# lucidrains/audiolm-pytorch

Measured on AMD Instinct MI355X. Metric: audio-tokens/sec fwd+bwd, CoarseTransformer d=1024 seq=2048, higher is better.
Workload: dtype bf16; 1 GPU; CoarseTransformer dim=1024 depth=6 heads=8 (MQA) num_coarse_quantizers=3 codebook=1024 semantic=500 residual_streams=4 flash_attn=True; per-GPU B=8, N=2048 (509 semantic + 512x3 coarse ids + eos/start); mask_prob=0.15; global_batch=8, seq_len=2048, parallelism=dp1

## Files before the change

audiolm-pytorch_amd/_lib.py:

```python
from __future__ import annotations

import ctypes
import os
from ctypes import c_float, c_int, c_longlong, c_ulonglong, c_void_p

_HERE = os.path.dirname(os.path.abspath(__file__))
LIB_PATH = os.environ.get('ALM_LIB_PATH') or os.path.join(_HERE, 'libaudiolm_hip.so')

_P, _I, _L, _F, _U = c_void_p, c_int, c_longlong, c_float, c_ulonglong

SIGNATURES = {
    'alm_gemm_bf16_nt': [_P, _P, _P, _P, _I, _I, _I, _L, _L, _L, _I, _I, _L, _L, _L, _L, _L, _L, _F, _I, _I, _P],
    'alm_gemm_bf16_nt_ws': [_P, _P, _P, _P, _I, _I, _I, _L, _L, _L, _I, _I, _L, _L, _L, _L, _L, _L, _F, _I, _I, _P, _L, _P],
    'alm_gemm_bf16_nt_inl': [_P, _P, _P, _P, _I, _I, _I, _L, _L, _L, _F, _I, _I, _I, _P, _L, _P],
    'alm_gemm_nt_plan': [_I, _I, _I, _I, _I, _P],
    'alm_gemm_nt_ws_bytes': [],
    'alm_gemm_splitk_slices': [_I, _I, _I, _I],
    'alm_gemm_splitk_ws_floats': [_I, _I, _I, _I],
    'alm_gemm_splitk_tile': [_I, _I, _I, _I],
    'alm_gemm_nt_tile_choice': [_I, _I, _I],
    'alm_gemm_tn_batched_plan': [_I, _I, _I, _I, _P],
    'alm_gemm_bf16_nt_splitk': [_P, _P, _P, _P, _I, _I, _I, _L, _L, _L, _I, _L, _L, _L, _F, _I, _P],
    'alm_gemm_bf16_tn_splitk': [_P, _P, _P, _P, _I, _I, _I, _L, _L, _L, _I, _L, _L, _L, _F, _I, _P],
    'alm_gemm_bf16_tn_batched': [_P, _P, _P, _P, _I, _I, _I, _L, _L, _L, _I, _I, _L, _L, _L, _L, _L, _L, _F, _I, _P],
    'alm_gemm_bf16_nt_group2': [_P, _P, _P, _I, _I, _I, _L, _L, _L, _P, _P, _P, _I, _I, _I, _L, _L, _L, _I, _P],
    'alm_gemm_bf16_nt_tile': [_P, _P, _P, _P, _I, _I, _I, _L, _L, _L, _F, _I, _I, _I, _P],
    'alm_transpose_bf16': [_P, _P, _I, _I, _L, _L, _I, _P],
    'alm_transpose_bf16_batched': [_P, _P, _I, _I, _L, _L, _I, _I, _L, _L, _P],
    'alm_pack_weights_multi': [_P, _I, _P],
    'alm_pack_weight': [_P, _I, _I, _L, _P, _L, _I, _I, _P, _L, _P],
    'alm_ln_partial_blocks': [_I],
    'alm_layernorm_fwd': [_P, _I, _L, _P, _P, _I, _L, _P, _L, _P, _P, _I, _I, _P],
    'alm_layernorm_bwd': [_P, _I, _L, _P, _I, _L, _P, _P, _P, _P, _L, _P, _I, _L, _P, _I, _I, _P],
    'alm_colsum': [_P, _I, _L, _I, _I, _P, _F, _I, _P, _P],
    'alm_colsum_chunks': [_I],
    'alm_colsum_partial': [_P, _L, _I, _I, _P, _P],
    'alm_geglu_fwd': [_P, _P, _L, _I, _P],
    'alm_geglu_bwd': [_P, _P, _P, _L, _I, _P],
    'alm_geglu_partial_blocks': [_I],
    'alm_geglu_ln_fwd': [_P, _L, _I, _P, _P, _L, _P, _P, _I, _I, _I, _P],
    'alm_geglu_ln_bwd': [_P, _L, _P, _L, _I, _P, _P, _P, _P, _P, _I, _I, _I, _P],
    'alm_mqa_attn_fwd': [_P, _L, _P, _L, _P, _L, _P, _P, _L, _P, _I, _I, _I, _I, _F, _F, _U, _P, _P],
    'alm_mqa_attn_bwd': [_P, _L, _P, _L, _P, _L, _P, _P, _L, _P, _P, _L, _P, _L, _P, _P, _L, _L, _P, _I, _I, _I, _I, _F, _F, _U, _P, _P],
    'alm_mqa_attn_bias_fwd': [_P, _L, _P, _L, _P, _L, _P, _P, _L, _P, _I, _I, _I, _I, _F, _P, _I, _P, _P, _P, _P, _F, _U, _P, _P],
    'alm_mqa_attn_bias_bwd': [_P, _L, _P, _L, _P, _L, _P, _P, _L, _P, _P, _L, _P, _L, _P, _P, _L, _L, _P, _I, _I, _I, _I, _F,
                              _P, _I, _P, _P, _P, _P, _P, _F, _U, _P, _P],
    'alm_attn_bias_part_rows': [_I, _I, _I],
    'alm_attn_bias_grad_reduce': [_P, _P, _I, _I, _I, _I, _F, _P],
    'alm_posmlp_in_fwd': [_P, _P, _P, _P, _P, _I, _I, _I, _P],
    'alm_posmlp_in_bwd_chunks': [_I],
    'alm_posmlp_in_bwd': [_P, _P, _P, _I, _I, _I, _P],
    'alm_silu_fwd': [_P, _P, _L, _P],
    'alm_silu_bwd': [_P, _P, _P, _L, _P],
    'alm_posmlp_out_fwd': [_P, _P, _P, _P, _P, _I, _I, _I, _F, _P],
    'alm_posmlp_out_bwd': [_P, _P, _P, _P, _P, _P, _I, _I, _I, _I, _F, _P],
    'alm_xattn_softmax_fwd': [_P, _L, _P, _P, _F, _P, _L, _P, _P, _P, _L, _I, _I, _I, _I, _I, _P],
    'alm_xattn_dbias': [_P, _L, _P, _L, _P, _P, _L, _I, _I, _I, _I, _P],
    'alm_xattn_combine': [_P, _L, _P, _P, _P, _L, _L, _I, _I, _P],
    'alm_xattn_softmax_bwd': [_P, _L, _P, _L, _P, _F, _P, _L, _I, _I, _I, _I, _P],
    'alm_xattn_delta': [_P, _L, _P, _L, _P, _I, _I, _I, _I, _P],
    'alm_value_residual_mix': [_P, _L, _P, _L, _P, _L, _L, _I, _P],
    'alm_kv_grad_pack': [_P, _P, _L, _I, _L, _P, _P, _L, _L, _I, _I, _P],
    'alm_forgetful_mask': [_P, _L, _P, _L, _I, _I, _I, _P],
    'alm_coarse_prepare': [_P, _L, _P, _L, _I, _I, _I, _L, _L, _L, _I, _I, _P, _P, _P, _P, _I, _P],
    'alm_semantic_prepare': [_P, _L, _I, _I, _L, _L, _P, _P, _I, _P],
    'alm_unique_consecutive_i64': [_P, _L, _I, _I, _I, _L, _L, _P, _L, _P, _P],
    'alm_fine_prepare': [_P, _L, _P, _L, _I, _I, _I, _L, _L, _I, _I, _I, _P, _P, _P],
    'alm_loss_combine': [_P, _P, _P, _P, _P, _P, _P, _P, _L, _L, _L, _L, _F, _F, _F, _F, _I, _L, _P, _P, _P],
    'alm_mqa_head_groups': [_I],
    'alm_mqa_bwd_parts': [_I, _I, _I],
    'alm_hc_coef_width': [_I],
    'alm_hc_partial_width': [_I, _I],
    'alm_hc_grads_width': [_I, _I],
    'alm_hc_partial_rows': [_I, _I, _I, _I, _L, _I],
    'alm_hc_fwd': [_P, _I, _I, _P, _L, _P, _P, _P, _P, _P, _P, _P, _P, _P, _P, _P, _L, _P, _L, _P, _P, _P, _P, _P, _I, _I, _I, _I, _I, _P],
    'alm_hc_bwd': [_P, _I, _I, _P, _L, _P, _L, _P, _L, _P, _P, _P, _P, _I, _P, _P, _P, _P, _P, _P, _P, _P, _P, _F, _P, _P, _L, _P, _P, _L, _P, _I, _I, _I, _I, _I, _P],
    'alm_hc_param_grads': [_P, _I, _P, _P, _P, _P, _I, _I, _P],
    'alm_hc_param_grads_batched': [_P, _P, _I, _P, _P, _P, _P, _P, _I, _I, _P],
    'alm_streams_expand': [_P, _P, _I, _I, _L, _P],
    'alm_streams_reduce': [_P, _P, _I, _I, _L, _P],
    'alm_residual_add': [_P, _P, _L, _P, _L, _I, _P],
    'alm_f32_to_bf16': [_P, _P, _P, _L, _L, _I, _P],
    'alm_add_f32': [_P, _P, _P, _L, _F, _P],
    'alm_embed_assemble': [_P, _P, _I, _P, _P, _P, _L, _I, _P, _P],
    'alm_embed_scatter_add': [_P, _P, _I, _P, _P, _P, _F, _L, _I, _P],
    'alm_embed_scatter_ws_floats': [_P, _I, _L, _I],
    'alm_embed_scatter_owned': [_P, _P, _I, _P, _P, _P, _F, _L, _I, _P, _P],
    'alm_gather_split_bf16': [_P, _L, _L, _P, _P, _P, _L, _L, _I, _P],
    'alm_gather_rows_bf16': [_P, _L, _P, _P, _L, _L, _I, _P],
    'alm_scatter_rows_bf16': [_P, _L, _P, _P, _L, _L, _I, _P],
    'alm_cross_entropy_fwd': [_P, _L, _P, _P, _P, _L, _I, _I, _P],
    'alm_cross_entropy_bwd': [_P, _L, _P, _P, _P, _P, _L, _L, _I, _I, _I, _P],
    'alm_reduce_sum': [_P, _L, _P, _F, _P],
    'alm_mqa_decode_attn': [_P, _L, _P, _L, _P, _L, _P, _L, _P, _L, _I, _I, _I, _I, _I, _F, _P, _I, _I, _I, _P, _P, _P, _P, _P, _P],
    'alm_opt_chunk_elems': [],
    'alm_opt_grad_sumsq': [_P, _I, _P, _I, _P, _P],
    'alm_opt_adam_step': [_P, _I, _P, _I, _F, _F, _F, _F, _I, _I, _P, _F, _P],
    'alm_opt_adam_pack_step': [_P, _I, _F, _F, _F, _F, _I, _I, _P, _F, _P],
    'alm_conv1d_packed_floats': [_I, _I, _I],
    'alm_conv1d_pack': [_P, _P, _I, _I, _I, _P],
    'alm_conv1d_causal': [_P, _P, _P, _P, _P, _I, _I, _I, _I, _I, _I, _I, _I, _I, _P],
    'alm_resunit_causal': [_P, _P, _P, _P, _P, _P, _I, _I, _I, _I, _I, _P],
    'alm_phase_interleave': [_P, _P, _I, _I, _I, _I, _P],
    'alm_rvq_decode': [_P, _L, _P, _P, _L, _I, _I, _I, _I, _P],
    'alm_rvq_padded_codes': [_I],
    'alm_rvq_padded_dim': [_I],
    'alm_rvq_pack': [_P, _P, _P, _I, _I, _I, _P],
    'alm_rvq_encode': [_P, _L, _P, _P, _P, _P, _L, _P, _L, _I, _I, _I, _I, _P],
    'alm_bct_to_btc': [_P, _P, _I, _I, _I, _P],
    'alm_resample_sinc': [_P, _L, _P, _L, _P, _I, _L, _L, _L, _I, _I, _I, _P],
    'alm_resample_sinc_bwd': [_P, _L, _P, _L, _P, _I, _L, _L, _L, _I, _I, _I, _P],
    'alm_hubert_conv0_chunks': [_L],
    'alm_hubert_conv0_stats': [_P, _L, _P, _P, _P, _I, _I, _L, _L, _I, _I, _F, _P],
    'alm_hubert_conv0_apply': [_P, _L, _P, _P, _P, _P, _P, _I, _I, _L, _L, _I, _I, _P],
    'alm_conv1d_valid': [_P, _P, _P, _P, _P, _I, _I, _I, _I, _I, _I, _I, _I, _I, _I, _P],
    'alm_layernorm_bct_split': [_P, _P, _P, _P, _I, _I, _I, _F, _P],
    'alm_mha_attn_fwd': [_P, _P, _I, _I, _I, _I, _F, _P],
    'alm_t5_embed': [_P, _P, _P, _I, _I, _L, _P, _P],
    'alm_t5_rmsnorm': [_P, _P, _P, _P, _I, _I, _F, _I, _P],
    'alm_t5_gate': [_P, _P, _L, _L, _I, _P],
    'alm_t5_attn_fwd': [_P, _P, _P, _P, _I, _I, _I, _I, _P],
    'alm_layernorm_bct': [_P, _P, _P, _P, _I, _I, _I, _F, _P],
    'alm_geglu_bct': [_P, _P, _I, _I, _I, _P],
    'alm_local_attn': [_P, _P, _P, _P, _P, _P, _P, _P, _I, _I, _I, _I, _I, _F, _P],
    'alm_conv1d_causal_pre': [_P, _P, _P, _P, _P, _I, _I, _I, _I, _I, _I, _I, _I, _I, _I, _P],
    'alm_lstm_launches': [_I, _I],
    'alm_lstm_seq': [_P, _P, _P, _P, _P, _P, _P, _P, _I, _I, _I, _I, _P],
    'alm_memset_zero': [_P, _L, _P],
    'alm_list_op_id': [ctypes.c_char_p],
    'alm_list_op_nargs': [_I],
    'alm_list_run': [_P, _I, _P, _P, _I, _P, _I, _P, _P],
}

_lib = None


class AlmError(RuntimeError):
    pass


def load(build_if_missing: bool = True):
    global _lib
    if _lib is not None:
        return _lib
    if build_if_missing and not os.environ.get('ALM_LIB_PATH'):
        from . import build as _build
        try:
            _build.build(verbose=False)
        except Exception as e:
            if not os.path.exists(LIB_PATH):
                raise ImportError(f'libaudiolm_hip.so is missing and could not be built: {e}') from e
            if not _build._fresh(_build._digest()):
                raise ImportError(f'libaudiolm_hip.so is stale (csrc/ or include/ changed since it was built) and could not be rebuilt: {e}') from e
# ... 55 lines not shown
```

audiolm-pytorch_amd/core.py:

```python
from __future__ import annotations

import os
import sys
from dataclasses import dataclass

import torch

from . import launchlist, ops, relpos, xattn

BF16, F32 = torch.bfloat16, torch.float32


@dataclass
class StackCfg:
    dim: int
    depth: int
    heads: int
    dim_head: int
    streams: int
    inner: int
    add_value_residual: bool
    grad_shrink_alpha: float
    residual_bf16: bool = False
    cross_attend: bool = False
# ... 462 lines not shown

class _SideStream:
    _streams = {}

    def __init__(self, dev, enabled=True):
        self.enabled = enabled and dev.type == 'cuda'
        if self.enabled:
            self.main = torch.cuda.current_stream(dev)
            key = (dev.type, dev.index, SIDE_STREAMS, self.main.cuda_stream)
            if key not in _SideStream._streams:
                _SideStream._streams[key] = [torch.cuda.Stream(device=dev) for _ in range(SIDE_STREAMS)]
            self.streams = _SideStream._streams[key]
            self.turn = 0

    def _issue(self, stream, fn, tensors):
        ev = torch.cuda.Event()
        ev.record(self.main)
        for t in tensors:
            t.record_stream(stream)
        with torch.cuda.stream(stream):
            stream.wait_event(ev)
            return fn()

    def run(self, fn, *tensors):
        if not self.enabled:
            return fn()
        stream = self.streams[self.turn % len(self.streams)]
        self.turn += 1
        return self._issue(stream, fn, tensors)

    def run_after_all(self, fn, *tensors):
        if not self.enabled:
            return fn()
        s0 = self.streams[0]
        for s in self.streams[1:]:
            ev = torch.cuda.Event()
            ev.record(s)
            s0.wait_event(ev)
        return self._issue(s0, fn, tensors)

    def join(self):
        if self.enabled:
            for s in self.streams:
                ev = torch.cuda.Event()
                ev.record(s)
                self.main.wait_event(ev)


ASYNC_WGRAD = os.environ.get('ALM_ASYNC_WGRAD', '1') != '0'
QKV_GROUP = {'0': 0, '1': 1}.get(os.environ.get('ALM_QKV_GROUP', 'auto'), -1)
QKV_GROUP_MAX_M = 8192
ASYNC_KV = os.environ.get('ALM_ASYNC_KV', '0') != '0'
DEFER_WGRAD = os.environ.get('ALM_DEFER_WGRAD', '1') != '0'
DEFER_MAX_BYTES = int(float(os.environ.get('ALM_DEFER_MAX_GB', '24')) * (1 << 30))


def deferred_bytes(cfg, M):
    return cfg.depth * M * (2 * cfg.dim + 2 * cfg.inner_pad + cfg.heads * cfg.dim_head + 2 * cfg.dim_head) * 2
DEFER_GROUPS = max(1, int(os.environ.get('ALM_DEFER_GROUPS', '1')))
DP_DEFER_GROUPS = max(0, int(os.environ.get('ALM_DP_DEFER_GROUPS', '2')))
_DPGS = os.environ.get('ALM_DP_GROUP_SIZES', '').replace(' ', '').lower()
DP_GROUP_SIZES = None if _DPGS == '' else (() if _DPGS == 'even' else tuple(int(v) for v in _DPGS.split(',') if v))


def dp_group_sizes(L, ngroups):
    if DP_GROUP_SIZES is not None:
        return DP_GROUP_SIZES
    return (L - 1, 1) if (ngroups == 2 and L >= 3) else ()
DEFER_GROUP_SIZES = tuple(int(v) for v in os.environ.get('ALM_DEFER_GROUP_SIZES', '').replace(' ', '').split(',') if v)


def group_starts(L, ngroups, sizes=()):
    if sizes:
        if sum(sizes) != L or min(sizes) < 1:
            raise ValueError(f'ALM_DP_GROUP_SIZES={sizes}: the group sizes must be positive and sum to the depth {L}')
        starts, top = [], L
        for n in sizes:
            top -= n
            starts.append(top)
        return sorted(starts)
    gsz = (L + ngroups - 1) // ngroups
    return list(range(0, L, gsz))
HC_BATCH_FINISH = os.environ.get('ALM_HC_BATCH_FINISH', '1') != '0'
DEFER_SMALL_LATE = os.environ.get('ALM_DEFER_SMALL_LATE', '1') != '0'
_DEBUG_DEFER_GROUPS_CAPTURE = 1
MICRO_ASYNC_WGRAD = os.environ.get('ALM_MICRO_ASYNC_WGRAD', '0') != '0'
SIDE_STREAMS = max(1, int(os.environ.get('ALM_SIDE_STREAMS', '1')))


TRACE = None


def _vgrad_mode(acc, mixed):
    return 0 if acc is None else (1 if mixed else 2)


def ff_backward(cfg, W, prm, sv, dY, side, want_trace=False, du_out=None):
    M, D = dY.shape
    I, Ip, dev = cfg.inner, cfg.inner_pad, dY.device
    (_, W1T), (_, W2T) = W['w1'], W['w2']
    run = side.run if side is not None else (lambda fn, *t: fn())
    dHN = _empty((M, Ip), BF16, dev)
    fa = sv['alpha']
    ops.gemm_nt(dY, W2T, dHN, alpha=fa)
    if sv['keep'] is not None:
        dHN.mul_(sv['keep'])
    deferred = du_out is not None
    dW2 = None
    if not deferred:
        dW2 = _empty((D, I), F32, dev)
        HNs, dYs = sv['HN'], dY
        run(lambda: ops.gemm_tn_splitk(dYs, HNs[:, :I], dW2, alpha=fa), dYs, HNs, dW2)
    dU, dg3 = ops.geglu_ln_bwd(dHN, sv['U'], prm['ln3'], sv['mean3'], sv['rstd3'], I, Ip, du_out=du_out)
    dXN = _empty((M, D), BF16, dev)
    ops.gemm_nt(dU, W1T, dXN)
    dW1 = None
    if not deferred:
        dW1 = _empty((2 * I, D), F32, dev)
        XNs = sv['XN']
        run(lambda: ops.gemm_tn_splitk(dU.view(M, 2, Ip).permute(1, 0, 2)[:, :, :I], XNs, dW1.view(2, I, D)), dU, XNs, dW1)
    return (dXN, dW1, dg3, dW2, dHN, dU) if want_trace else (dXN, dW1, dg3, dW2)


def stack_backward(dhn, mask_u8, flat, cfg: StackCfg, cache: WeightCache, saved, on_layer_grads=None, bias=None, async_wgrad=True, dx_scale=1.0):
    B, N = saved['B'], saved['N']
    D, S, H, dh = cfg.dim, cfg.streams, cfg.heads, cfg.dim_head
    M = B * N
    I, Ip = cfg.inner, cfg.inner_pad
    dev = dhn.device
    ppl = params_per_layer(S, cfg.cross_attend)
    grads = [None] * len(flat)
    side = _SideStream(dev, ASYNC_WGRAD and async_wgrad)
    rdt = BF16 if (cfg.residual_bf16 and S > 1) else F32
    ctx = saved['ctx']
    brs = saved['branches']
    scale = float(dh) ** -0.5

    dxs, dgam = ops.layernorm_bwd(dhn, saved['xs'], saved['fmean'], saved['frstd'], flat[-1])
    grads[-1] = dgam
    multi = cfg.add_value_residual and cfg.depth > 1
    acc_v0 = ops._new_zeros((M, dh), dtype=F32, device=dev) if multi else None
    acc_vp0 = ops._new_zeros((B * ctx.m, dh), dtype=F32, device=dev) if (multi and cfg.prefix) else None
    acc_vc0 = ops._new_zeros((B * ctx.m, dh), dtype=F32, device=dev) if (multi and cfg.cross_attend) else None
    dctx = None
    dense = isinstance(bias, relpos.DenseBias)
    dtbl_part = ops.attn_bias_part(B, N, H, bias.tbl.shape[1], dev) if (bias is not None and not dense) else None
    ddense = torch.zeros_like(bias.tbl) if dense else None
    dR, bcast = dxs, S > 1
    dY = dbeta = None
    stk = saved.get('stk')
    bst = None
    if stk is not None:
        L = cfg.depth
        bst = dict(dYat=_empty((L, M, D), BF16, dev), dYff=_empty((L, M, D), BF16, dev), dU=_empty((L, M, 2 * Ip), BF16, dev),
                   dQ=_empty((L, M, H * dh), BF16, dev), dKV=_empty((L, M, 2 * dh), BF16, dev))

    def dy_slot(br):
        return None if bst is None else bst['dYat' if br['kind'] == 'attn' else 'dYff'][br['layer']]
    if S > 1:
        h = ops.hc_bwd(dxs, B, S, N, D, bcast=True, y_prev=brs[-1]['Y'], coef_prev=brs[-1]['coef'], r_dtype=rdt, dy_out=dy_slot(brs[-1]))
        dY, dbeta = h['dy'], h['dbeta']

    wg = None
    if bst is not None:
        L = cfg.depth
        ngroups = _DEBUG_DEFER_GROUPS_CAPTURE if (dev.type == 'cuda' and torch.cuda.is_current_stream_capturing()) else (
            DEFER_GROUPS if on_layer_grads is None else max(1, DP_DEFER_GROUPS))
        ngroups = min(ngroups, L)
        capturing = dev.type == 'cuda' and torch.cuda.is_current_stream_capturing()
        starts = group_starts(L, ngroups, () if capturing else (dp_group_sizes(L, ngroups) if on_layer_grads is not None else DEFER_GROUP_SIZES))
        ngroups = len(starts)
        on_group = getattr(on_layer_grads, 'on_group', None)
        group_buffer = getattr(on_layer_grads, 'group_buffer', None)
        wg = True
        wshape = dict(dW1=(2, I, D), dW2=(1, D, I), dWo=(1, D, H * dh), dWq=(1, H * dh, D), dWkv=(1, 2 * dh, D))
        hc_n_ = 7 if S > 1 else 0
        wslot = dict(dWq=hc_n_ + 1, dWkv=hc_n_ + 2, dWo=hc_n_ + 3, dW1=(hc_n_ + 4) + hc_n_ + 1, dW2=(hc_n_ + 4) + hc_n_ + 3)

        big_kinds, small_kinds = ('dW1', 'dW2'), ('dWo', 'dWq', 'dWkv')
        late = DEFER_SMALL_LATE and ngroups > 1
        handed = set()

        def group_outputs(l0, l1, kinds, late_kinds):
            views = None
            if group_buffer is not None:
                views = group_buffer(l0, l1, [wslot[k] for k in kinds], [wslot[k] for k in late_kinds],
                                     [wslot[k] for k in small_kinds] if (late and not late_kinds) else [])
            if views is not None:
                return {k: v.view(-1, *wshape[k]) for k, v in zip(tuple(kinds) + tuple(late_kinds), views)}
            out = {k: _empty((l1 - l0,) + wshape[k], F32, dev) for k in kinds}
            out.update({k: _empty((L,) + wshape[k], F32, dev) for k in late_kinds})
            return out

        def launch_group(l0):
            l1 = ([s_ for s_ in starts if s_ > l0] + [L])[0]
            last = l0 == 0
            kinds = big_kinds if late else big_kinds + small_kinds
            late_kinds = small_kinds if (late and last) else ()
            wgg = group_outputs(l0, l1, kinds, late_kinds)
            operands = dict(dW1=lambda a, b: (bst['dU'][a:b].view(b - a, M, 2, Ip).permute(0, 2, 1, 3)[..., :I], stk['XNff'][a:b].unsqueeze(1)),
                            dW2=lambda a, b: (bst['dYff'][a:b].unsqueeze(1), stk['HN'][a:b][..., :I].unsqueeze(1)),
                            dWo=lambda a, b: (bst['dYat'][a:b].unsqueeze(1), stk['AO'][a:b].unsqueeze(1)),
                            dWq=lambda a, b: (bst['dQ'][a:b].unsqueeze(1), stk['XNat'][a:b].unsqueeze(1)),
                            dWkv=lambda a, b: (bst['dKV'][a:b].unsqueeze(1), stk['Xat'][a:b].unsqueeze(1)))
            jobs = [operands[k](l0, l1) + (wgg[k],) for k in kinds] + [operands[k](0, L) + (wgg[k],) for k in late_kinds]
            for At, Bt, C in jobs:
                if ngroups > 1 or on_layer_grads is not None:
                    side.run(lambda At=At, Bt=Bt, C=C: ops.gemm_tn_batched(At, Bt, C), At, Bt, C)
                else:
                    ops.gemm_tn_batched(At, Bt, C)
            for k in kinds:
                for l in range(l0, l1):
                    g_ = wgg[k][l - l0]
                    grads[l * ppl + wslot[k]] = g_.view(2 * I, D) if k == 'dW1' else g_[0]
            for k in late_kinds:
                for l in range(L):
                    grads[l * ppl + wslot[k]] = wgg[k][l, 0]
            if on_layer_grads is not None:
                layers = list(range((L if late_kinds else l1) - 1, l0 - 1, -1))
                per_layer = []
                for l in layers:
                    gl = [g if (l * ppl + j) not in handed else None for j, g in enumerate(grads[l * ppl:(l + 1) * ppl])]
                    handed.update(l * ppl + j for j, g in enumerate(gl) if g is not None)
                    per_layer.append(gl)
                live = [g for gl in per_layer for g in gl if g is not None]
                if on_group is not None:
                    side.run_after_all(lambda: on_group(layers, per_layer), *live)
                else:
                    def hand_off():
                        for l, gl in zip(layers, per_layer):
                            on_layer_grads(l, gl)
                    side.run_after_all(hand_off, *live)

    hc_pending = []

    def finish_hc():
        if not hc_pending:
            return
        for (first_, ip_, _, rec_), g_ in zip(hc_pending, ops.hc_param_grads_batched([t[2] for t in hc_pending], S, D)):
            for j, k in enumerate(HC_KEYS):
                grads[first_ + j] = g_[k]
            grads[ip_] = g_['ln']
            if rec_ is not None:
                rec_['hc_grads'] = dict(g_)
        hc_pending.clear()

    def add_ctx(g):
        nonlocal dctx
        dctx = g if dctx is None else ops.add_f32(dctx, g)

    LW, LW_layer = None, -1
    for bi in reversed(range(len(brs))):
        sv = brs[bi]
        kind, l, first = sv['kind'], sv['layer'], sv['first']
        if l != LW_layer:
            branches = _split_layer(flat[l * ppl:(l + 1) * ppl], S, cfg.cross_attend)
            LW, LW_layer = layer_weights(cache, l, branches, I, Ip), l
            prms = {k: (d, f) for k, d, f in branches}
        prm = prms[kind][0]
        hc_n = 7 if S > 1 else 0
        ip = first + hc_n
        if S == 1:
            dY = ops.f32_to_bf16(dR, out=dy_slot(sv))
        extra = None
        W = LW[kind]
        if kind == 'ff':
            dXN, dW1, dg3, dW2, dHN, dU = ff_backward(cfg, W, prm, sv, dY, side, want_trace=True, du_out=bst['dU'][l] if bst is not None else None)
            grads[ip + 1], grads[ip + 2], grads[ip + 3] = dW1, dg3, dW2
            rec = dict(dY=dY, dHN=dHN, dU=dU, dXN=dXN, dW1=dW1, dg3=dg3, dW2=dW2) if TRACE is not None else None
        elif kind == 'cross':
            (_, WqT), (_, WkvT), (_, WoT) = W['wq'], W['wkv'], W['wo']
            m = ctx.m
            dAO = _empty((M, H * dh), BF16, dev)
            oa = sv['oalpha']
            dYs = dY if sv['okeep'] is None else dY * sv['okeep']
            ops.gemm_nt(dYs, WoT, dAO, alpha=oa)
            dWo = _empty((D, H * dh), F32, dev)
            AOs = sv['AO']
            side.run(lambda: ops.gemm_tn_splitk(dYs, AOs, dWo, alpha=oa), dYs, AOs, dWo)
            nd = xattn.attn_delta(sv['AO'], dAO, B, N, H, dh)
            dQ, dke, dve = xattn.extra_attn_bwd(sv['Q'], dAO, sv['xs'], nd, B, N, H, dh, scale)
            dnull = torch.stack((dke[:, 0].sum(0), dve[:, 0].sum(0))).reshape(2, 1, dh)
            dkv32 = torch.cat((dke[:, 1:].reshape(B * m, dh), dve[:, 1:].reshape(B * m, dh)), dim=1).contiguous()
            dKVc = ops.kv_grad_pack(dkv32, acc_vc0, _vgrad_mode(acc_vc0, sv['cmixed']), dh)
            dXN = _empty((M, D), BF16, dev)
            ops.gemm_nt(dQ, WqT, dXN)
            dWq = _empty((H * dh, D), F32, dev)
            XNs = sv['XN']
            side.run(lambda: ops.gemm_tn_splitk(dQ, XNs, dWq), dQ, XNs, dWq)
            dCN = _empty((B * m, cfg.dim_context), BF16, dev)
            ops.gemm_nt(dKVc, WkvT, dCN)
            dWkv = _empty((2 * dh, cfg.dim_context), F32, dev)
            CNs = sv['CN']
            side.run(lambda: ops.gemm_tn_splitk(dKVc, CNs, dWkv), dKVc, CNs, dWkv)
            dc, dgc = ops.layernorm_bwd(dCN, ctx.x, sv['cmean'], sv['crstd'], prm['ctx_ln'])
            add_ctx(dc)
            grads[ip + 1], grads[ip + 2], grads[ip + 3], grads[ip + 4], grads[ip + 5] = dgc, dnull, dWq, dWkv, dWo
            rec = dict(dY=dY) if TRACE is not None else None
        else:
            (_, WqT), (_, WkvT), (_, WoT) = W['wq'], W['wkv'], W['wo']
            dAO = _empty((M, H * dh), BF16, dev)
            oa = sv['oalpha']
            dYs = dY if sv['okeep'] is None else dY * sv['okeep']
            ops.gemm_nt(dYs, WoT, dAO, alpha=oa)
            dWo = dWq = dWkv = None
            if bst is None:
                dWo = _empty((D, H * dh), F32, dev)
                AOs = sv['AO']
                side.run(lambda: ops.gemm_tn_splitk(dYs, AOs, dWo, alpha=oa), dYs, AOs, dWo)
            pd, dseed, dseed_dev = sv['drop']
            KV = sv['KV']
            dense_pre = None
            if dense:
                nd = xattn.attn_delta(sv['AO'], dAO, B, N, H, dh)
                mpre = ctx.m if sv['pre'] is not None else 0
                dbl = torch.empty((H, N, mpre + N), dtype=F32, device=dev)
                dQ, dke, dve = xattn.extra_attn_bwd(sv['Q'], dAO, sv['dense'], nd, B, N, H, dh, scale, dbias=dbl)
                ddense += dbl[:, :, mpre:]
                if mpre:
                    dense_pre = (dke[:, :mpre], dve[:, :mpre])
                    dke, dve = dke[:, mpre:], dve[:, mpre:]
                dkv32 = torch.cat((dke.reshape(M, dh), dve.reshape(M, dh)), dim=1).contiguous()
            else:
                dQ, dkv32 = ops.mqa_attn_bwd(sv['Q'], KV[:, :dh], sv['V'], mask_u8, sv['AO'], sv['LSE'], dAO, B, N, H, dh, bias=bias, dtbl_part=dtbl_part,
                                             dropout_p=pd, seed=dseed, dq_out=bst['dQ'][l] if bst is not None else None, seed_dev=dseed_dev)
            dKV = ops.kv_grad_pack(dkv32, acc_v0, _vgrad_mode(acc_v0, sv['mixed']), dh, out=bst['dKV'][l] if bst is not None else None)
            dKVp = None
            pre = sv['pre']
            if pre is not None:
                m = ctx.m
                if dense_pre is not None:
                    dke, dve = dense_pre
                else:
                    nd = xattn.attn_delta(sv['AO'], dAO, B, N, H, dh)
                    dQ, dke, dve = xattn.extra_attn_bwd(sv['Q'], dAO, pre['xs'], nd, B, N, H, dh, scale, dq=dQ)
                dkvp32 = torch.cat((dke.reshape(B * m, dh), dve.reshape(B * m, dh)), dim=1).contiguous()
                dKVp = ops.kv_grad_pack(dkvp32, acc_vp0, _vgrad_mode(acc_vp0, pre['pmixed']), dh)
                dcp = _empty((B * m, D), F32, dev)
                ops.gemm_nt(dKVp, WkvT, dcp)
                add_ctx(dcp)
            dXN = _empty((M, D), BF16, dev)
            extra = _empty((M, D), BF16, dev)
            ops.gemm_nt_group2(dQ, WqT, dXN, dKV, WkvT, extra)
            if bst is None:
                dWq = _empty((H * dh, D), F32, dev)
                XNs = sv['XN']
                side.run(lambda: ops.gemm_tn_splitk(dQ, XNs, dWq), dQ, XNs, dWq)
                dWkv = _empty((2 * dh, D), F32, dev)
                Xs, cx = sv['X'], (ctx.x if dKVp is not None else None)

                def wkv_grad():
                    ops.gemm_tn_splitk(dKV, Xs, dWkv)
                    if dKVp is not None:
                        ops.gemm_tn_splitk(dKVp, cx, dWkv, accumulate=True)
                side.run(wkv_grad, *[t for t in (dKV, Xs, dWkv, dKVp, cx) if t is not None])
            grads[ip + 1], grads[ip + 2], grads[ip + 3] = dWq, dWkv, dWo
            rec = dict(dY=dY, dAO=dAO, dQ=dQ, dkv32=dkv32, dKV=dKV, dXN=dXN, extra=extra, dWq=dWq, dWkv=dWkv, dWo=dWo) if TRACE is not None else None

        prev = brs[bi - 1] if bi > 0 else None
        if S > 1:
            py, pc = (prev['Y'], prev['coef']) if prev is not None else (None, None)
            h = ops.hc_bwd(dR, B, S, N, D, bcast=bcast, dxn=dXN, extra=extra, mean=sv['mean'], rstd=sv['rstd'], ln_gamma=prm['ln'], R=sv['R'],
                           coef=sv['coef'], dbeta=dbeta, hc=prm['hc'], y_prev=py, coef_prev=pc, r_bcast=sv['r_bcast'], sum_only=prev is None,
                           r_dtype=rdt, dsum_scale=dx_scale if prev is None else 1.0, dy_out=dy_slot(prev) if prev is not None else None,
                           defer_grads=wg is not None and HC_BATCH_FINISH)
            if rec is not None:
                rec.update(kind=kind, layer=l, dR_in=dR, dR_in_bcast=bcast, dbeta_in=dbeta, dR_out=h['dsum'] if prev is None else h['dR'], sum_only=prev is None,
                           dY_prev=h['dy'], dbeta_prev=h['dbeta'], hc_grads=dict(h['grads']) if h['grads'] is not None else None)
                TRACE.append(rec)
            dR, dY, dbeta, bcast = (h['dsum'] if prev is None else h['dR']), h['dy'], h['dbeta'], False
            if h['grads'] is None:
                hc_pending.append((first, ip, h['part'], rec))
            else:
                for j, k in enumerate(HC_KEYS):
                    grads[first + j] = h['grads'][k]
                grads[ip] = h['grads']['ln']
        else:
            dX, dgl = ops.layernorm_bwd(dXN, sv['R'], sv['mean'], sv['rstd'], prm['ln'], extra=extra)
            if rec is not None:
                rec.update(kind=kind, layer=l, dR_in=dR, dX=dX, dln=dgl)
                TRACE.append(rec)
            dR = ops.add_f32(dR, dX, dx_scale if prev is None else 1.0)
            grads[ip] = dgl
        sv.clear()
        if wg is not None and (prev is None or prev['layer'] != l) and l in starts:
            finish_hc()
            launch_group(l)
        if on_layer_grads is not None and wg is None and (prev is None or prev['layer'] != l):
            base = l * ppl
            side.run_after_all(lambda: on_layer_grads(l, grads[base:base + ppl]), *[g for g in grads[base:base + ppl] if g is not None])

    finish_hc()
    dx = dR.view(B, N, D)
    dtbl = ddense if dense else (ops.attn_bias_grad_reduce(dtbl_part, B, N, H) if bias is not None else None)
    side.join()
    return dx, grads, dtbl, dctx


_MICRO_STREAMS = {}


def _micro_stream(dev):
    key = (dev.type, dev.index)
    if key not in _MICRO_STREAMS:
        _MICRO_STREAMS[key] = torch.cuda.Stream(device=dev)
    return _MICRO_STREAMS[key]


def _halves(t, h):
    return (None, None) if t is None else (t[:h], t[h:])


class TransformerStackFn(torch.autograd.Function):

    @staticmethod
    def forward(ctx, x, mask_u8, cfg, cache, opts, bias, tbl, context, *flat):
        hooks = opts.get('hook')
        need = bool(opts.get('grad', True)) and (any(t.requires_grad for t in flat) or x.requires_grad or (tbl is not None and tbl.requires_grad)
                                                 or (context is not None and context.requires_grad))
        xin = x.detach().contiguous().to(F32)
        bias = bias.detached() if bias is not None else None
        flat_d = flat
        B = xin.shape[0]
        cx = None
        if context is not None:
            m = context.shape[1]
            cm = opts.get('context_mask')
            cm = None if cm is None else cm.to(torch.bool).contiguous().view(torch.uint8)
            cx = Context(context.detach().to(BF16).reshape(B * m, -1).contiguous(), cm, B, m)
        ctx.ctx_meta = None if context is None else (context.shape, context.dtype)
        micro = int(opts.get('micro', 1))
        if micro == 2 and (B % 2 or B < 2 or opts.get('kv_out') is not None or opts.get('decode') is not None or hooks is not None):
            micro = 1
        ctx.micro = micro
        dseed = None
        if float(opts.get('attn_dropout', 0.)) > 0. and xin.is_cuda and torch.cuda.is_current_stream_capturing():
            seed_state = graph_seed_state(xin.device)
            seed_state.add_(2 * cfg.depth)
            dseed = (0, seed_state.clone())
        if micro == 1:
            defer = DEFER_WGRAD and (hooks is None or DP_DEFER_GROUPS > 0)
            plan = None
            if (launchlist.ENABLED and hooks is None and cx is None and opts.get('kv_out') is None and opts.get('decode') is None and TRACE is None
                    and float(opts.get('ff_dropout', 0.)) == 0. and float(opts.get('attn_dropout', 0.)) == 0. and not isinstance(bias, relpos.DenseBias)
                    and xin.is_cuda and not torch.cuda.is_current_stream_capturing()):
                plan = launchlist.plan_for(sys.modules[__name__], xin, mask_u8, cfg, need, bias, len(flat_d), defer, cfg.grad_shrink_alpha)
            if plan is not None:
                hn, saved = launchlist.forward(sys.modules[__name__], plan, xin, mask_u8, flat_d, cfg, cache, need, bias, defer)
            else:
                hn, saved = stack_forward(xin, mask_u8, flat_d, cfg, cache, need, bias, kv_out=opts.get('kv_out'), decode=opts.get('decode'), ctx=cx,
                                          ff_dropout=float(opts.get('ff_dropout', 0.)), attn_dropout=float(opts.get('attn_dropout', 0.)),
                                          defer_wgrad=defer, drop_seed=dseed)
        else:
            S, ppl, h = cfg.streams, params_per_layer(cfg.streams, cfg.cross_attend), B // 2
            for l in range(cfg.depth):
                layer_weights(cache, l, _split_layer(flat_d[l * ppl:(l + 1) * ppl], S, cfg.cross_attend), cfg.inner, cfg.inner_pad)
            cur, s2 = torch.cuda.current_stream(xin.device), _micro_stream(xin.device)
            (xa, xb), (ma, mb) = _halves(xin, h), _halves(mask_u8, h)
            ca = cb = None
            if cx is not None:
                (cma, cmb) = _halves(cx.mask, h)
                ca, cb = Context(cx.x[:h * cx.m], cma, h, cx.m), Context(cx.x[h * cx.m:], cmb, B - h, cx.m)
            s2.wait_stream(cur)
            adp = float(opts.get('attn_dropout', 0.))
            hna, sva = stack_forward(xa, ma, flat_d, cfg, cache, need, bias, ctx=ca, ff_dropout=float(opts.get('ff_dropout', 0.)), attn_dropout=adp, drop_seed=dseed)
            xb.record_stream(s2)
            with torch.cuda.stream(s2):
                hnb, svb = stack_forward(xb, mb, flat_d, cfg, cache, need, bias, ctx=cb, ff_dropout=float(opts.get('ff_dropout', 0.)), attn_dropout=adp,
                                         drop_seed=None if dseed is None else (cfg.depth, dseed[1]))
            cur.wait_stream(s2)
            hnb.record_stream(cur)
            hn = torch.cat((hna, hnb), dim=0)
            saved = (sva, svb)
        ctx.saved, ctx.cfg, ctx.cache, ctx.mask, ctx.hooks, ctx.bias = saved, cfg, cache, mask_u8, hooks, bias
        ctx.flat = flat
# ... 46 lines not shown
```

audiolm-pytorch_amd/csrc/attention.hip:

```cpp
#include <type_traits>

#include "common.hpp"
#include "../../include/audiolm_hip.h"

namespace {

constexpr int DH = 64;
constexpr float LOG2E = 1.4426950408889634f;
constexpr float RESCALE_THR = 8.0f;
constexpr unsigned OOB = 0x80000000u;
constexpr int HPB = 4;

typedef __attribute__((address_space(3))) void lds_void;

__device__ __forceinline__ int fsw(int row) { return (((row >> 1) & 1) << 2) | (((row >> 3) & 1) << 1) | ((row >> 2) & 1); }

typedef __attribute__((ext_vector_type(4))) float lds_f4v;
typedef __attribute__((ext_vector_type(4))) int lds_i4v;
__device__ __forceinline__ float4 lds_ld_f4(const float* p) {
    const lds_f4v v = *reinterpret_cast<const lds_f4v*>(p);
    return make_float4(v[0], v[1], v[2], v[3]);
}
__device__ __forceinline__ int4 lds_ld_i4(const int* p) {
    const lds_i4v v = *reinterpret_cast<const lds_i4v*>(p);
    return make_int4(v[0], v[1], v[2], v[3]);
}

__device__ __forceinline__ bf16x8 nat_frag(const unsigned char* tile, int row, int frow, int ks, int lh) {
    return *reinterpret_cast<const bf16x8*>(tile + row * 128 + ((((ks << 1) | lh) ^ frow) << 4));
}

struct TrOff { unsigned o[2][2]; };
__device__ __forceinline__ TrOff make_troff(int lane) {
    TrOff t;
    const int g = lane >> 4, s = lane & 15;
    const int rr = 4 * (g >> 1) + (s >> 2);
#pragma unroll
    for (int db = 0; db < 2; ++db)
#pragma unroll
        for (int r = 0; r < 2; ++r) {
            const int row = 8 * r + rr;
            const int ch = db * 4 + (g & 1) * 2 + ((s & 3) >> 1);
            t.o[db][r] = (unsigned)(row * 128 + ((ch ^ fsw(row)) << 4) + (s & 1) * 8);
        }
    return t;
}
__device__ __forceinline__ bf16x8 tr_frag(const unsigned char* tile, int k16, const TrOff& t, int db) {
    const unsigned char* base = tile + k16 * 128;
    return __builtin_shufflevector(lds_tr16(base + t.o[db][0]), lds_tr16(base + t.o[db][1]), 0, 1, 2, 3, 4, 5, 6, 7);
}

__device__ __forceinline__ bf16x8 pack8(const f32x16& v, int s) {
    typedef __attribute__((ext_vector_type(8))) float f32x8;
    typedef __attribute__((ext_vector_type(8))) __bf16 hbf16x8;
    f32x8 f;
#pragma unroll
    for (int j = 0; j < 8; ++j) f[j] = v[8 * s + j];
    return __builtin_bit_cast(bf16x8, __builtin_convertvector(f, hbf16x8));
}

__device__ __forceinline__ bf16x8 zero8() {
    bf16x8 r;
#pragma unroll
    for (int j = 0; j < 8; ++j) r[j] = 0;
    return r;
}

__device__ __forceinline__ bf16x8 gload8(const bf16_t* p, bool ok) {
    if (!ok) return zero8();
    return *reinterpret_cast<const bf16x8*>(p);
}

struct AttnParams {
    const bf16_t* q; const bf16_t* k; const bf16_t* v; const uint8_t* mask;
    bf16_t* o; float* lse;
    const bf16_t* dout; const float* ndelta; const float* nlse;
    bf16_t* dq; float* dk; float* dv;
    long long ldq, ldk, ldv, ldo, lddo, lddq, lddk, part_stride;
    int B, N, H, HG;
    int dkv_split;
    float scale;
    const float* tbl; const int* qkey4; const int* kkey4; const int* qattr; const int* kattr; float* dtbl_part;
    int LT;
    unsigned drop_thr; float drop_scale; unsigned seed_lo, seed_hi;
    const unsigned long long* seed_dev;
};

__device__ __forceinline__ unsigned mix32(unsigned x) {
    x ^= x >> 16; x *= 0x7feb352du; x ^= x >> 15; x *= 0x846ca68bu; x ^= x >> 16;
    return x;
}
__device__ __forceinline__ unsigned drop_salt(const AttnParams& p, int b, int head) {
    unsigned lo = p.seed_lo, hi = p.seed_hi;
    if (p.seed_dev) {
        const unsigned long long s = (((unsigned long long)hi << 32) | lo) + *p.seed_dev;
        lo = (unsigned)(s & 0xffffffffu);
        hi = (unsigned)(s >> 32);
    }
    return mix32(lo ^ mix32(hi + (unsigned)(b * p.H + head) * 0x9E3779B9u));
}
__device__ __forceinline__ bool drop_keep(unsigned salt, int qi, int kj, int N, unsigned thr) {
    return mix32(((unsigned)qi * (unsigned)N + (unsigned)kj) ^ salt) >= thr;
}

constexpr int WCAP = 1024;

template <bool SP>
__device__ __forceinline__ float bias_at(const __amdgpu_buffer_rsrc_t& rsT, int kq4, int kk4, int aq, int ak) {
    int voff = kq4 - kk4;
    if (SP) voff = (aq & ak) ? 0 : voff;
    return __uint_as_float(__builtin_amdgcn_raw_buffer_load_b32(rsT, voff, 0, 0));
}

__device__ __forceinline__ int wave_or(int v) {
#pragma unroll
    for (int o = 32; o > 0; o >>= 1) v |= __shfl_xor(v, o, 64);
    return __builtin_amdgcn_readfirstlane(v);
}

__device__ __forceinline__ float lse_log2(float l) { return l == -INFINITY ? INFINITY : l * LOG2E; }

__device__ __forceinline__ int drow(int r, int lh) { return (r & 3) + 8 * (r >> 2) + 4 * lh; }

struct BlockId { int blk, hg, b; };
__device__ __forceinline__ BlockId decode_block(int L, int nblk, int HG, int B, bool heavy_is_high, bool pair_on_cu) {
    BlockId r;
    const int combos = HG * B;
    if (pair_on_cu) {
        int p, ncl, half, xcd;
        if ((combos & 7) == 0) { xcd = L & 7; p = L >> 3; ncl = combos >> 3; half = 32; }
        else { xcd = -1; p = L; ncl = combos; half = 256; }
        const int W = ncl * nblk, M2 = min(W, 2 * half);
        const int g = (p < half || p >= M2) ? p : M2 - 1 - (p - half);
        const int rank = g / ncl, cl = g - rank * ncl;
        const int combo = xcd >= 0 ? cl * 8 + xcd : cl;
        r.hg = combo % HG;
        r.b = combo / HG;
        r.blk = heavy_is_high ? nblk - 1 - rank : rank;
        return r;
    }
    int idx, combo;
    if ((combos & 7) == 0) {
        const int xcd = L & 7, j = L >> 3;
        const int cl = j / nblk;
        idx = j % nblk;
        combo = cl * 8 + xcd;
    } else {
        idx = L % nblk;
        combo = L / nblk;
    }
    r.hg = combo % HG;
    r.b = combo / HG;
    r.blk = heavy_is_high ? nblk - 1 - idx : idx;
    return r;
}

template <int NP>
__device__ __forceinline__ void dma_tile(const __amdgpu_buffer_rsrc_t& rs, unsigned char* img, int first, int step, int lane, int row0, unsigned ld_bytes,
                                         unsigned col_bytes) {
#pragma unroll
    for (int i = 0; i < NP; ++i) {
        const int piece = first + i * step;
        const int row = piece * 8 + (lane >> 3);
        const int c = (lane & 7) ^ fsw(row);
        const unsigned vo = (unsigned)(row0 + row) * ld_bytes + col_bytes + (unsigned)c * 16u;
        __builtin_amdgcn_raw_ptr_buffer_load_lds(rs, (lds_void*)(img + piece * 1024), 16, vo, 0, 0, 0);
    }
}
// ... 300 lines not shown
            const float l = lse[idx];
            nlse[idx] = (l == -INFINITY) ? -INFINITY : -l * inv_scale;
        }
    }
}

template <bool BIAS, bool DROP = false>
__global__ __launch_bounds__(256, 2) void mqa_bwd_dq_kernel(AttnParams p) {
    extern __shared__ __attribute__((aligned(1024))) unsigned char smem[];
    float* kbias = reinterpret_cast<float*>(smem + 32768);
    int* kk4s = reinterpret_cast<int*>(smem + 32768 + 512);
    int* kas = kk4s + 128;
    int* kmm = kas + 128;
    float* wins = reinterpret_cast<float*>(smem + 32768 + 512 + 1024 + 64);

    const int nqb = (p.N + 63) / 64;
    const BlockId id = decode_block(blockIdx.x, nqb, p.HG, p.B, true, true);
    const int qblk = id.blk, b = id.b;
    const int q0 = qblk * 64;
    const int t = threadIdx.x;
    const int lane = t & 63;
    const int wave = __builtin_amdgcn_readfirstlane(t >> 6);
    const int head = id.hg * HPB + wave;
    const bool active = head < p.H;
    const int lr = lane & 31, lh = lane >> 5;
    const float c2 = p.scale * LOG2E;
    const unsigned dsalt = DROP ? drop_salt(p, b, active ? head : 0) : 0u;

    const bf16_t* kbase = p.k + (long long)b * p.N * p.ldk;
    const bf16_t* vbase = p.v + (long long)b * p.N * p.ldv;
    const auto rsK = __builtin_amdgcn_make_buffer_rsrc(const_cast<bf16_t*>(kbase), 0, (int)(((long long)(p.N - 1) * p.ldk + DH) * 2), 0x00020000);
    const auto rsV = __builtin_amdgcn_make_buffer_rsrc(const_cast<bf16_t*>(vbase), 0, (int)(((long long)(p.N - 1) * p.ldv + DH) * 2), 0x00020000);
    const uint8_t* mrow = p.mask ? p.mask + (long long)b * p.N : nullptr;

    struct KeySide { int raw; };
    auto load_side = [&](int tile) {
        KeySide ks{1};
        if (t < 64) {
            const int key = tile * 64 + t;
            ks.raw = key < p.N;
            if (ks.raw && mrow) ks.raw = mrow[key];
        }
        return ks;
    };
    auto stage = [&](unsigned char* __restrict__ img, int tile, int buf, const KeySide& ks) {
        dma_tile<2>(rsK, img, wave, 4, lane, tile * 64, (unsigned)(p.ldk * 2), 0);
        dma_tile<2>(rsV, img + 8192, wave, 4, lane, tile * 64, (unsigned)(p.ldv * 2), 0);
        if (t < 64) {
            int raw = ks.raw;
            asm volatile("" : "+v"(raw));
            kbias[buf * 64 + t] = raw ? 0.f : -INFINITY;
            if (BIAS) {
                const int kc = min(tile * 64 + t, p.N - 1);
                const int kv = p.kkey4[kc];
                kk4s[buf * 64 + t] = kv;
                const int ka = p.kattr[kc];
                kas[buf * 64 + t] = ka;
                const int ko = wave_or(ka);
                int mn = kv, mx = kv;
#pragma unroll
                for (int o = 32; o > 0; o >>= 1) {
                    mn = min(mn, __shfl_xor(mn, o, 64));
                    mx = max(mx, __shfl_xor(mx, o, 64));
                }
                if (t == 0) { kmm[buf * 4] = mn; kmm[buf * 4 + 1] = mx; kmm[buf * 4 + 2] = ko; }
            }
        }
    };

    bf16x8 qf[2][4], dof[2][4];
    float lse2[2], dlt[2];
#pragma unroll
    for (int qb = 0; qb < 2; ++qb) {
        const int qi = q0 + qb * 32 + lr;
        const bool ok = active && qi < p.N;
        const bf16_t* qp = p.q + ((long long)b * p.N + qi) * p.ldq + head * DH;
        const bf16_t* dp = p.dout + ((long long)b * p.N + qi) * p.lddo + head * DH;
#pragma unroll
        for (int ks = 0; ks < 4; ++ks) {
            qf[qb][ks] = gload8(qp + ks * 16 + lh * 8, ok);
            dof[qb][ks] = gload8(dp + ks * 16 + lh * 8, ok);
        }
        lse2[qb] = ok ? lse_log2(p.lse[((long long)b * p.H + head) * p.N + qi]) : INFINITY;
        dlt[qb] = ok ? p.ndelta[((long long)b * p.H + head) * p.N + qi] : 0.f;
    }

    int kq4[2] = {0, 0}, aq[2] = {0, 0}, qmin4[2] = {0, 0}, qmax4[2] = {0, 0};
    __amdgpu_buffer_rsrc_t rsT = rsK;
    float* win = wins + wave * WCAP;
    float* part = nullptr;
    if (BIAS) {
        rsT = __builtin_amdgcn_make_buffer_rsrc(const_cast<float*>(p.tbl + (long long)(active ? head : 0) * p.LT), 0, p.LT * 4, 0x00020000);
        part = p.dtbl_part + ((((long long)b * p.HG + id.hg) * nqb + qblk) * HPB + wave) * p.LT;
#pragma unroll
        for (int qb = 0; qb < 2; ++qb) {
            const int qc = min(q0 + qb * 32 + lr, p.N - 1);
            kq4[qb] = p.qkey4[qc];
            aq[qb] = p.qattr[qc];
            int mn = kq4[qb], mx = kq4[qb];
#pragma unroll
            for (int o = 16; o > 0; o >>= 1) {
                mn = min(mn, __shfl_xor(mn, o, 64));
                mx = max(mx, __shfl_xor(mx, o, 64));
            }
            qmin4[qb] = __builtin_amdgcn_readfirstlane(mn);
            qmax4[qb] = __builtin_amdgcn_readfirstlane(mx);
        }
        for (int e = lane; e < WCAP; e += 64) win[e] = 0.f;
    }
    const int aq_or = BIAS ? wave_or(aq[0] | aq[1]) : 0;

    f32x16 dq[2][2];
#pragma unroll
    for (int i = 0; i < 2; ++i)
#pragma unroll
        for (int j = 0; j < 2; ++j)
#pragma unroll
            for (int r = 0; r < 16; ++r) dq[i][j][r] = 0.f;

    const int frow = fsw(lr);
    const TrOff troff = make_troff(lane);
    const int ntiles = qblk + 1;

    KeySide side = load_side(0);
    stage(smem, 0, 0, side);
    side = load_side(1);
    __syncthreads();

    auto step = [&](unsigned char* __restrict__ nimg, const unsigned char* __restrict__ Kt, int tile) {
        const int buf = tile & 1;
        if (tile + 1 < ntiles) stage(nimg, tile + 1, buf ^ 1, side);
        side = load_side(tile + 2);
        if (active) {
            const unsigned char* Vt = Kt + 8192;
            const float* kbs = kbias + buf * 64;
#pragma unroll
            for (int qb = 0; qb < 2; ++qb) {
                f32x16 st[2], dpt[2];
                const bool sp_tile = BIAS && (aq_or & __builtin_amdgcn_readfirstlane(kmm[buf * 4 + 2])) != 0;
                auto init_scores = [&](auto spc) {
                    constexpr bool SP = decltype(spc)::value;
#pragma unroll
                    for (int kb = 0; kb < 2; ++kb)
#pragma unroll
                        for (int g = 0; g < 4; ++g) {
                            const float4 bv = lds_ld_f4(kbs + kb * 32 + 8 * g + 4 * lh);
                            const float bvv[4] = {bv.x, bv.y, bv.z, bv.w};
                            if (BIAS) {
                                const int4 kk = lds_ld_i4(kk4s + buf * 64 + kb * 32 + 8 * g + 4 * lh);
                                int4 ka = make_int4(0, 0, 0, 0);
                                if (SP) ka = lds_ld_i4(kas + buf * 64 + kb * 32 + 8 * g + 4 * lh);
                                const int kkv[4] = {kk.x, kk.y, kk.z, kk.w}, kav[4] = {ka.x, ka.y, ka.z, ka.w};
#pragma unroll
                                for (int c = 0; c < 4; ++c) st[kb][4 * g + c] = bvv[c] + bias_at<SP>(rsT, kq4[qb], kkv[c], aq[qb], kav[c]);
                            } else {
#pragma unroll
                                for (int c = 0; c < 4; ++c) st[kb][4 * g + c] = bvv[c];
                            }
#pragma unroll
                            for (int c = 0; c < 4; ++c) dpt[kb][4 * g + c] = 0.f;
                        }
                };
                if (sp_tile) init_scores(std::true_type{});
                else init_scores(std::false_type{});
#pragma unroll
                for (int ks = 0; ks < 4; ++ks)
#pragma unroll
// ... 376 lines not shown
            } else {
#pragma unroll
            for (int qb = 0; qb < 2; ++qb)
#pragma unroll
                for (int r = 0; r < 16; ++r) {
                    const int qq = q0 + qb * 32 + drow(r, lh);
                    float pv = __builtin_amdgcn_exp2f(s[qb][r] * c2);
                    if (DIAG ? key_eff > qq : !kvalid) pv = 0.f;
                    if (DROP) {
                        const bool kp = drop_keep(dsalt, qq, key, p.N, p.drop_thr);
                        const float nd = rowt[64 + qb * 32 + drow(r, lh)];
                        dp[qb][r] = pv * ((kp ? dp[qb][r] * p.drop_scale : 0.f) + nd);
                        s[qb][r] = kp ? pv : 0.f;
                    } else {
                        s[qb][r] = pv;
                        dp[qb][r] *= pv;
                    }
                }
            }
            DKV_PROBE_T(2);
#pragma unroll
            for (int qb = 0; qb < 2; ++qb)
#pragma unroll
                for (int st = 0; st < 2; ++st) {
                    const bf16x8 pf = pack8(s[qb], st);
                    const bf16x8 dsf = pack8(dp[qb], st);
#pragma unroll
                    for (int db = 0; db < 2; ++db) {
                        const bf16x8 dotf = tr_frag(Dt, qb * 32 + st * 16, troff, db);
                        dvt[db] = __builtin_amdgcn_mfma_f32_32x32x16_bf16(dotf, pf, dvt[db], 0, 0, 0);
                        const bf16x8 qtf = tr_frag(Qt, qb * 32 + st * 16, troff, db);
                        dkt[db] = __builtin_amdgcn_mfma_f32_32x32x16_bf16(qtf, dsf, dkt[db], 0, 0, 0);
                    }
                }
            }
            DKV_PROBE_T(3);
        }
    };
    int qfirst = q_lo;
    if (part == 0) {
        step(smem + STG, smem, kblk, std::true_type{}, std::true_type{});
        __syncthreads();
        qfirst = kblk + 1;
    }
    DKV_PROBE_T(4);
    constexpr bool PEEL_LAST = !DROP && !BIAS;
#pragma unroll 1
    for (int qt = qfirst; qt + (PEEL_LAST ? 1 : 0) < q_hi; ++qt) {
        const int buf = (qt - q_lo) & 1;
        step(smem + (buf ^ 1) * STG, smem + buf * STG, qt, std::false_type{}, std::true_type{});
        __syncthreads();
        DKV_PROBE_T(4);
    }
    if (PEEL_LAST && q_hi - 1 >= qfirst) {
        const int buf = (q_hi - 1 - q_lo) & 1;
        step(smem + (buf ^ 1) * STG, smem + buf * STG, q_hi - 1, std::false_type{}, std::false_type{});
        __syncthreads();
        DKV_PROBE_T(4);
    }
    DKV_PROBE_FLUSH(blockIdx.x * 8 + wave, q_hi - q_lo);

    constexpr int RS = 33, RW = 64 * RS;
    float* red = reinterpret_cast<float*>(smem);
    for (int pass = 0; pass < 2; ++pass) {
        if (pass) __syncthreads();
        const f32x16* acc = pass == 0 ? dkt : dvt;
        if (active) {
#pragma unroll
            for (int db = 0; db < 2; ++db)
#pragma unroll
                for (int r = 0; r < 16; ++r) red[wave * RW + (db * 32 + drow(r, lh)) * RS + lr] = acc[db][r];
        }
        __syncthreads();
        float* outp = (pass == 0 ? p.dk : p.dv) + (long long)id.hg * p.part_stride;
        const float sc = pass == 0 ? p.scale : (DROP ? p.drop_scale : 1.f);
        const int nh = min(NH, p.H - hgq * NH);
        for (int e = t; e < 64 * 64; e += NT) {
            const int kk = e >> 6, d = e & 63;
            const int half = kk >> 5, kl = kk & 31;
            float sum = 0.f;
            for (int hh = 0; hh < nh; ++hh) sum += red[(hh * 2 + half) * RW + d * RS + kl];
            if (kblk * 64 + kk < p.N) {
                const bool kv_ok = !p.mask || p.mask[(long long)b * p.N + kblk * 64 + kk] != 0;
                outp[((long long)b * p.N + kblk * 64 + kk) * p.lddk + d] = kv_ok ? sum * sc : 0.f;
            }
        }
    }
}

__global__ __launch_bounds__(256) void bias_grad_reduce_kernel(const float* __restrict__ part, float* __restrict__ dtbl, int B, int HG, int nqb,
                                                               int H, int LT, float scale) {
    const int t = blockIdx.x * 256 + threadIdx.x;
    const int h = blockIdx.y;
    if (t >= LT) return;
    const int hg = h / HPB, w = h % HPB;
    float s0 = 0.f, s1 = 0.f;
    for (int b = 0; b < B; ++b) {
        const float* pp = part + ((((long long)b * HG + hg) * nqb) * HPB + w) * LT + t;
        int qb = 0;
        for (; qb + 1 < nqb; qb += 2) {
            s0 += pp[(long long)qb * HPB * LT];
            s1 += pp[(long long)(qb + 1) * HPB * LT];
        }
        if (qb < nqb) s0 += pp[(long long)qb * HPB * LT];
    }
    dtbl[(long long)h * LT + t] = (s0 + s1) * scale;
}

}

static int check_attn(int B, int N, int H, long long ldq, long long ldk, long long ldv, long long ldo) {
    if (B <= 0 || N <= 0 || H <= 0 || H > 64) return ALM_ERR_UNSUPPORTED;
    if ((ldq & 7) || (ldk & 7) || (ldv & 7) || (ldo & 3)) return ALM_ERR_BAD_ARG;
    if ((long long)N * ldq * 2 >= 0x7fffffffLL || (long long)N * ldk * 2 >= 0x7fffffffLL || (long long)N * ldv * 2 >= 0x7fffffffLL) return ALM_ERR_UNSUPPORTED;
    const long long ldmax = ldq > ldk ? (ldq > ldv ? ldq : ldv) : (ldk > ldv ? ldk : ldv);
    if ((long long)(N + 64) * (ldmax > ldo ? ldmax : ldo) * 2 >= 0xffffffffLL) return ALM_ERR_UNSUPPORTED;
    return 0;
}

extern "C" int alm_mqa_head_groups(int H) { return (H + HPB - 1) / HPB; }

static int dkv_heads_per_block(int B, int N, int H) {
    static const int env_nh = [] { const char* e = getenv("ALM_ATTN_DKV_NH"); return e ? atoi(e) : 0; }();
    if (env_nh == 2 || env_nh == 4) return env_nh;
    (void)B; (void)H;
    return N >= 8192 ? 2 : HPB;
}
static int dkv_split(int B, int N, int H, int nh) {
    static const int env_sp = [] { const char* e = getenv("ALM_ATTN_DKV_SPLIT"); return e ? atoi(e) : 0; }();
    if (env_sp == 1 || env_sp == 2) return env_sp;
    const long long wgs = (long long)((N + 63) / 64) * ((H + nh - 1) / nh) * B;
    return (N > 64 && 2 * wgs <= 256) ? 2 : 1;
}
extern "C" int alm_mqa_bwd_parts(int B, int N, int H) {
    const int nh = dkv_heads_per_block(B, N, H);
    return ((H + nh - 1) / nh) * dkv_split(B, N, H, nh);
}

struct BiasArgs { const float* tbl; int LT; const int* qkey4; const int* kkey4; const int* qattr; const int* kattr; float* dtbl_part; };

static int check_bias(const BiasArgs& ba, bool bwd) {
    if (!ba.tbl) return 0;
    if (ba.LT < 2 || ba.LT > (1 << 28) || !ba.qkey4 || !ba.kkey4 || !ba.qattr || !ba.kattr || (bwd && !ba.dtbl_part)) return ALM_ERR_BAD_ARG;
    if (((uintptr_t)ba.qkey4 & 15) || ((uintptr_t)ba.qattr & 15)) return ALM_ERR_BAD_ARG;
    return 0;
}

static bool set_dropout(AttnParams& p, float dropout_p, unsigned long long seed, const void* seed_dev) {
    p.seed_dev = nullptr;
    if (!(dropout_p > 0.f)) return false;
    p.seed_dev = reinterpret_cast<const unsigned long long*>(seed_dev);
    const double thr = (double)dropout_p * 4294967296.0;
    p.drop_thr = thr >= 4294967295.0 ? 4294967295u : (unsigned)thr;
    p.drop_scale = 1.f / (1.f - dropout_p);
    p.seed_lo = (unsigned)(seed & 0xffffffffu);
    p.seed_hi = (unsigned)(seed >> 32);
    return true;
}

static int attn_fwd_impl(const void* q, long long ldq, const void* k, long long ldk, const void* v, long long ldv,
                         const unsigned char* mask, void* o, long long ldo, float* lse, int B, int N, int H, int dim_head,
                         float scale, const BiasArgs& ba, float dropout_p, unsigned long long seed, const void* seed_dev, void* stream) {
    if (dropout_p < 0.f || dropout_p >= 1.f) return ALM_ERR_BAD_ARG;
    if (dim_head != DH) return ALM_ERR_UNSUPPORTED;
    int rc = check_attn(B, N, H, ldq, ldk, ldv, ldo);
    if (rc) return rc;
    if (((uintptr_t)q & 15) || ((uintptr_t)k & 15) || ((uintptr_t)v & 15) || ((uintptr_t)o & 7)) return ALM_ERR_BAD_ARG;
    AttnParams p{};
    p.q = (const bf16_t*)q; p.k = (const bf16_t*)k; p.v = (const bf16_t*)v; p.mask = mask; p.o = (bf16_t*)o; p.lse = lse;
    p.ldq = ldq; p.ldk = ldk; p.ldv = ldv; p.ldo = ldo; p.B = B; p.N = N; p.H = H; p.HG = alm_mqa_head_groups(H); p.scale = scale;
    rc = check_bias(ba, false);
    if (rc) return rc;
    p.tbl = ba.tbl; p.LT = ba.LT; p.qkey4 = ba.qkey4; p.kkey4 = ba.kkey4; p.qattr = ba.qattr; p.kattr = ba.kattr;
    const int npair = ((N + 31) / 32 + 1) / 2;
    const bool drop = set_dropout(p, dropout_p, seed, seed_dev);
    static const int qb2_minn = [] { const char* e = getenv("ALM_ATTN_FWD_QB2_MINN"); return e ? atoi(e) : 0; }();
    if (qb2_minn > 0 && N >= qb2_minn && !drop && !p.tbl) {
        hipLaunchKernelGGL((mqa_fwd_kernel<false, 2>), dim3(((N + 63) / 64) * p.HG * B), dim3(256), FWD_LDS<false>, (hipStream_t)stream, p);
        ALM_LAUNCH_CHECK();
        return 0;
    }
    if (drop) {
        if (p.tbl) hipLaunchKernelGGL((mqa_fwd_kernel<true, 1, true>), dim3(npair * p.HG * B), dim3(256), FWD_LDS<true>, (hipStream_t)stream, p);
        else hipLaunchKernelGGL((mqa_fwd_kernel<false, 1, true>), dim3(npair * p.HG * B), dim3(256), FWD_LDS<false>, (hipStream_t)stream, p);
    } else if (p.tbl) hipLaunchKernelGGL((mqa_fwd_kernel<true, 1>), dim3(npair * p.HG * B), dim3(256), FWD_LDS<true>, (hipStream_t)stream, p);
    else hipLaunchKernelGGL((mqa_fwd_kernel<false, 1>), dim3(npair * p.HG * B), dim3(256), FWD_LDS<false>, (hipStream_t)stream, p);
    ALM_LAUNCH_CHECK();
    return 0;
}

static int attn_bwd_impl(const void* q, long long ldq, const void* k, long long ldk, const void* v, long long ldv,
                         const unsigned char* mask, const void* o, long long ldo, const float* lse, const void* dout, long long lddo,
                         void* dq, long long lddq, float* dk, float* dv, long long lddk, long long part_stride, float* delta, int B,
                         int N, int H, int dim_head, float scale, const BiasArgs& ba, float dropout_p, unsigned long long seed, const void* seed_dev, void* stream) {
    if (dim_head != DH) return ALM_ERR_UNSUPPORTED;
    if (dropout_p < 0.f || dropout_p >= 1.f) return ALM_ERR_BAD_ARG;
    int rc = check_attn(B, N, H, ldq, ldk, ldv, ldo);
    if (rc) return rc;
    if ((lddo & 7) || (lddq & 3) || (long long)N * lddo * 2 >= 0x7fffffffLL) return ALM_ERR_BAD_ARG;
    if ((long long)(N + 64) * lddo * 2 >= 0xffffffffLL) return ALM_ERR_UNSUPPORTED;
    rc = check_bias(ba, true);
    if (rc) return rc;
    if (((uintptr_t)q & 15) || ((uintptr_t)k & 15) || ((uintptr_t)v & 15) || ((uintptr_t)dout & 15) || ((uintptr_t)dq & 7)) return ALM_ERR_BAD_ARG;
    hipStream_t st = (hipStream_t)stream;
    float* ndelta = delta;
    float* nlse = delta + (long long)B * H * N;
    hipLaunchKernelGGL(attn_delta_kernel, dim3(((long long)B * N + 3) / 4), dim3(256), 0, st, (const bf16_t*)o, ldo, (const bf16_t*)dout, lddo, lse,
                       ndelta, nlse, 1.0f / scale, B, N, H);
    AttnParams p{};
    p.q = (const bf16_t*)q; p.k = (const bf16_t*)k; p.v = (const bf16_t*)v; p.mask = mask; p.lse = const_cast<float*>(lse);
    p.dout = (const bf16_t*)dout; p.ndelta = ndelta; p.nlse = nlse; p.dq = (bf16_t*)dq; p.dk = dk; p.dv = dv;
    p.ldq = ldq; p.ldk = ldk; p.ldv = ldv; p.ldo = ldo; p.lddo = lddo; p.lddq = lddq; p.lddk = lddk; p.part_stride = part_stride;
    p.B = B; p.N = N; p.H = H; p.HG = alm_mqa_head_groups(H); p.scale = scale;
    p.tbl = ba.tbl; p.LT = ba.LT; p.qkey4 = ba.qkey4; p.kkey4 = ba.kkey4; p.qattr = ba.qattr; p.kattr = ba.kattr; p.dtbl_part = ba.dtbl_part;
    const int nqb = (N + 63) / 64;
    const bool drop = set_dropout(p, dropout_p, seed, seed_dev);
    if (drop) {
        if (p.tbl) hipLaunchKernelGGL((mqa_bwd_dq_kernel<true, true>), dim3(nqb * p.HG * B), dim3(256), DQ_LDS<true>, st, p);
        else hipLaunchKernelGGL((mqa_bwd_dq_kernel<false, true>), dim3(nqb * p.HG * B), dim3(256), DQ_LDS<false>, st, p);
    } else if (p.tbl) hipLaunchKernelGGL(mqa_bwd_dq_kernel<true>, dim3(nqb * p.HG * B), dim3(256), DQ_LDS<true>, st, p);
    else hipLaunchKernelGGL(mqa_bwd_dq_kernel<false>, dim3(nqb * p.HG * B), dim3(256), DQ_LDS<false>, st, p);
    const int nh = dkv_heads_per_block(B, N, H);
    p.HG = (H + nh - 1) / nh;
    p.dkv_split = dkv_split(B, N, H, nh);
    auto launch_dkv = [&](auto kern, int threads, int lds) -> hipError_t {
        static const void* done[8] = {nullptr, nullptr, nullptr, nullptr, nullptr, nullptr, nullptr, nullptr};
        const void* fn = reinterpret_cast<const void*>(kern);
        bool seen = false;
        for (int i = 0; i < 8; ++i) seen = seen || done[i] == fn;
        if (!seen) {
            const hipError_t e = hipFuncSetAttribute(fn, hipFuncAttributeMaxDynamicSharedMemorySize, lds);
            if (e != hipSuccess) return e;
            for (int i = 0; i < 8; ++i) if (done[i] == nullptr) { done[i] = fn; break; }
        }
        hipLaunchKernelGGL(kern, dim3(nqb * p.HG * p.dkv_split * B), dim3(threads), lds, st, p);
        return hipSuccess;
    };
    hipError_t le;
    if (nh == 2) {
        constexpr int LDS2 = 2 * 2 * 16384 + 2 * 2 * 512;
        if (drop) le = p.tbl ? launch_dkv(mqa_bwd_dkv_kernel<true, true, 2>, 256, LDS2) : launch_dkv(mqa_bwd_dkv_kernel<false, true, 2>, 256, LDS2);
        else le = p.tbl ? launch_dkv(mqa_bwd_dkv_kernel<true, false, 2>, 256, LDS2) : launch_dkv(mqa_bwd_dkv_kernel<false, false, 2>, 256, LDS2);
    } else {
        constexpr int LDS4 = 131072 + 4096;
        if (drop) le = p.tbl ? launch_dkv(mqa_bwd_dkv_kernel<true, true, 4>, 512, LDS4) : launch_dkv(mqa_bwd_dkv_kernel<false, true, 4>, 512, LDS4);
        else le = p.tbl ? launch_dkv(mqa_bwd_dkv_kernel<true, false, 4>, 512, LDS4) : launch_dkv(mqa_bwd_dkv_kernel<false, false, 4>, 512, LDS4);
    }
    if (le != hipSuccess) return (int)le;
    ALM_LAUNCH_CHECK();
    return 0;
}

extern "C" int alm_mqa_attn_fwd(const void* q, long long ldq, const void* k, long long ldk, const void* v, long long ldv,
                                const unsigned char* mask, void* o, long long ldo, float* lse, int B, int N, int H, int dim_head,
                                float scale, float dropout_p, unsigned long long seed, const void* seed_dev, void* stream) {
    return attn_fwd_impl(q, ldq, k, ldk, v, ldv, mask, o, ldo, lse, B, N, H, dim_head, scale, BiasArgs{}, dropout_p, seed, seed_dev, stream);
}

extern "C" int alm_mqa_attn_bwd(const void* q, long long ldq, const void* k, long long ldk, const void* v, long long ldv,
                                const unsigned char* mask, const void* o, long long ldo, const float* lse, const void* dout, long long lddo,
                                void* dq, long long lddq, float* dk, float* dv, long long lddk, long long part_stride, float* delta, int B,
                                int N, int H, int dim_head, float scale, float dropout_p, unsigned long long seed, const void* seed_dev, void* stream) {
    return attn_bwd_impl(q, ldq, k, ldk, v, ldv, mask, o, ldo, lse, dout, lddo, dq, lddq, dk, dv, lddk, part_stride, delta, B, N, H, dim_head,
                         scale, BiasArgs{}, dropout_p, seed, seed_dev, stream);
}

extern "C" int alm_mqa_attn_bias_fwd(const void* q, long long ldq, const void* k, long long ldk, const void* v, long long ldv,
                                     const unsigned char* mask, void* o, long long ldo, float* lse, int B, int N, int H, int dim_head,
                                     float scale, const float* tbl, int LT, const int* qkey4, const int* kkey4, const int* qattr,
                                     const int* kattr, float dropout_p, unsigned long long seed, const void* seed_dev, void* stream) {
    if (!tbl) return ALM_ERR_BAD_ARG;
    return attn_fwd_impl(q, ldq, k, ldk, v, ldv, mask, o, ldo, lse, B, N, H, dim_head, scale, BiasArgs{tbl, LT, qkey4, kkey4, qattr, kattr, nullptr},
                         dropout_p, seed, seed_dev, stream);
}

extern "C" int alm_mqa_attn_bias_bwd(const void* q, long long ldq, const void* k, long long ldk, const void* v, long long ldv,
                                     const unsigned char* mask, const void* o, long long ldo, const float* lse, const void* dout,
                                     long long lddo, void* dq, long long lddq, float* dk, float* dv, long long lddk, long long part_stride,
                                     float* delta, int B, int N, int H, int dim_head, float scale, const float* tbl, int LT, const int* qkey4,
                                     const int* kkey4, const int* qattr, const int* kattr, float* dtbl_part, float dropout_p,
                                     unsigned long long seed, const void* seed_dev, void* stream) {
    if (!tbl) return ALM_ERR_BAD_ARG;
    return attn_bwd_impl(q, ldq, k, ldk, v, ldv, mask, o, ldo, lse, dout, lddo, dq, lddq, dk, dv, lddk, part_stride, delta, B, N, H, dim_head,
                         scale, BiasArgs{tbl, LT, qkey4, kkey4, qattr, kattr, dtbl_part}, dropout_p, seed, seed_dev, stream);
}

extern "C" int alm_attn_bias_part_rows(int B, int N, int H) { return B * alm_mqa_head_groups(H) * ((N + 63) / 64) * HPB; }

extern "C" int alm_attn_bias_grad_reduce(const float* dtbl_part, float* dtbl, int B, int N, int H, int LT, float scale, void* stream) {
    if (B <= 0 || N <= 0 || H <= 0 || LT <= 0) return ALM_ERR_BAD_ARG;
    hipLaunchKernelGGL(bias_grad_reduce_kernel, dim3((LT + 255) / 256, H), dim3(256), 0, (hipStream_t)stream, dtbl_part, dtbl, B,
                       alm_mqa_head_groups(H), (N + 63) / 64, H, LT, scale);
    ALM_LAUNCH_CHECK();
    return 0;
}

#if defined(ALM_ATTN_PROBE) || defined(ALM_DKV_PROBE)
extern "C" int alm_attn_probe_read(unsigned long long* host, int n) {
    return (int)hipMemcpyFromSymbol(host, HIP_SYMBOL(g_attn_probe), sizeof(unsigned long long) * n);
}
#endif
```

audiolm-pytorch_amd/csrc/launchlist.hip:

```cpp
#include <hip/hip_runtime.h>
#include <stdint.h>
#include <string.h>

#include <utility>
#include <vector>

#include "../../include/audiolm_hip.h"

namespace {

template <class T> struct Slot;
template <> struct Slot<int> { static int get(uint64_t v) { return (int)(int64_t)v; } };
template <> struct Slot<long long> { static long long get(uint64_t v) { return (long long)v; } };
template <> struct Slot<unsigned long long> { static unsigned long long get(uint64_t v) { return (unsigned long long)v; } };
template <> struct Slot<float> {
    static float get(uint64_t v) {
        uint32_t u = (uint32_t)v;
        float f;
        memcpy(&f, &u, 4);
        return f;
    }
};
template <class T> struct Slot<T*> { static T* get(uint64_t v) { return (T*)(uintptr_t)v; } };

template <class... A, size_t... I> int invoke(int (*f)(A...), const uint64_t* a, std::index_sequence<I...>) { return f(Slot<A>::get(a[I])...); }
template <class... A> int call_packed(int (*f)(A...), const uint64_t* a) { return invoke(f, a, std::index_sequence_for<A...>{}); }
template <class... A> constexpr int arity(int (*)(A...)) { return (int)sizeof...(A); }

struct Op {
    const char* name;
    int nargs;
    int (*thunk)(const uint64_t*);
};

#define ALM_OP(fn) {#fn, arity(fn), [](const uint64_t* a) -> int { return call_packed(fn, a); }}

__global__ __launch_bounds__(256) void zero_bytes_kernel(unsigned char* __restrict__ p, long long n) {
    const uintptr_t a = reinterpret_cast<uintptr_t>(p);
    const long long head = (long long)((16 - (a & 15)) & 15) < n ? (long long)((16 - (a & 15)) & 15) : n;
    const long long nvec = (n - head) / 16;
    uint4* v = reinterpret_cast<uint4*>(p + head);
    for (long long i = (long long)blockIdx.x * 256 + threadIdx.x; i < nvec; i += (long long)gridDim.x * 256) v[i] = make_uint4(0, 0, 0, 0);
    if (blockIdx.x == 0) {
        if ((long long)threadIdx.x < head) p[threadIdx.x] = 0;
        const long long tail0 = head + nvec * 16;
        if (tail0 + threadIdx.x < n && threadIdx.x < 16) p[tail0 + threadIdx.x] = 0;
    }
}

const Op OPS[] = {
    ALM_OP(alm_memset_zero),
    ALM_OP(alm_gemm_bf16_nt),
    ALM_OP(alm_gemm_bf16_nt_ws),
    ALM_OP(alm_gemm_bf16_nt_group2),
    ALM_OP(alm_gemm_bf16_nt_splitk),
    ALM_OP(alm_gemm_bf16_tn_splitk),
    ALM_OP(alm_gemm_bf16_tn_batched),
    ALM_OP(alm_layernorm_fwd),
    ALM_OP(alm_layernorm_bwd),
    ALM_OP(alm_colsum),
    ALM_OP(alm_colsum_partial),
    ALM_OP(alm_geglu_ln_fwd),
    ALM_OP(alm_geglu_ln_bwd),
    ALM_OP(alm_mqa_attn_fwd),
    ALM_OP(alm_mqa_attn_bwd),
    ALM_OP(alm_mqa_attn_bias_fwd),
    ALM_OP(alm_mqa_attn_bias_bwd),
    ALM_OP(alm_attn_bias_grad_reduce),
    ALM_OP(alm_value_residual_mix),
    ALM_OP(alm_kv_grad_pack),
    ALM_OP(alm_hc_fwd),
    ALM_OP(alm_hc_bwd),
    ALM_OP(alm_hc_param_grads),
    ALM_OP(alm_hc_param_grads_batched),
    ALM_OP(alm_streams_expand),
    ALM_OP(alm_streams_reduce),
    ALM_OP(alm_residual_add),
    ALM_OP(alm_f32_to_bf16),
    ALM_OP(alm_add_f32),
};
constexpr int NOPS = (int)(sizeof(OPS) / sizeof(OPS[0]));

}

extern "C" {

int alm_memset_zero(void* ptr, long long bytes, void* stream) {
    if (bytes < 0 || (bytes > 0 && ptr == nullptr)) return ALM_ERR_BAD_ARG;
    if (bytes == 0) return 0;
    const long long chunks = (bytes + 15) / 16 + 1;
    const long long blocks = (chunks + 255) / 256;
    hipLaunchKernelGGL(zero_bytes_kernel, dim3((unsigned)(blocks < 65535 * 16 ? blocks : 65535 * 16)), dim3(256), 0, (hipStream_t)stream,
                       reinterpret_cast<unsigned char*>(ptr), bytes);
    return (int)hipGetLastError();
}

int alm_list_op_id(const char* name) {
    if (name == nullptr) return -1;
    for (int i = 0; i < NOPS; ++i)
        if (strcmp(OPS[i].name, name) == 0) return i;
    return -1;
}

int alm_list_op_nargs(int op) { return (op >= 0 && op < NOPS) ? OPS[op].nargs : -1; }

int alm_list_run(const AlmListEntry* entries, int n, const unsigned long long* slots, const unsigned short* reloc, int nslots, const unsigned long long* bases,
                 int nbases, void* stream, int* failed_at) {
    if (failed_at) *failed_at = -1;
    if (n < 0 || nslots < 0 || nbases < 0 || (n > 0 && entries == nullptr) || (nslots > 0 && (slots == nullptr || reloc == nullptr)) || (nbases > 0 && bases == nullptr))
        return ALM_ERR_BAD_ARG;
    static thread_local std::vector<uint64_t> r;
    r.resize((size_t)nslots);
    for (int i = 0; i < nslots; ++i) {
        const unsigned k = reloc[i];
        if (k == ALM_LIST_LITERAL) r[i] = slots[i];
        else if (k == ALM_LIST_STREAM) r[i] = (uint64_t)(uintptr_t)stream;
        else if (k == ALM_LIST_HOST_PTRS || k == ALM_LIST_HOST_INTS) r[i] = 0;
        else if ((int)k <= nbases) r[i] = bases[k - 1] + slots[i];
        else return ALM_ERR_BAD_ARG;
    }
    for (int i = 0; i < nslots; ++i) {
        const unsigned k = reloc[i];
        if (k != ALM_LIST_HOST_PTRS && k != ALM_LIST_HOST_INTS) continue;
        const uint64_t at = slots[i];
        if (at >= (uint64_t)nslots) return ALM_ERR_BAD_ARG;
        r[i] = (uint64_t)(uintptr_t)(k == ALM_LIST_HOST_PTRS ? (const void*)&r[at] : (const void*)&slots[at]);
    }
    for (int e = 0; e < n; ++e) {
        const AlmListEntry& en = entries[e];
        if (en.op < 0 || en.op >= NOPS || en.nargs != OPS[en.op].nargs || en.first < 0 || en.first + en.nargs > nslots) {
            if (failed_at) *failed_at = e;
            return ALM_ERR_BAD_ARG;
        }
        const int rc = OPS[en.op].thunk(r.data() + en.first);
        if (rc != 0) {
            if (failed_at) *failed_at = e;
            return rc;
        }
    }
    return 0;
}

}
```

audiolm-pytorch_amd/csrc/norm_act.hip:

```cpp
#include "common.hpp"
#include "../../include/audiolm_hip.h"

namespace {

constexpr float LN_EPS = 1e-5f;

__device__ __forceinline__ float4 load4(const float* p) { return *reinterpret_cast<const float4*>(p); }
__device__ __forceinline__ float4 load4(const bf16_t* p) {
    const uint2 u = *reinterpret_cast<const uint2*>(p);
    return make_float4(__uint_as_float(u.x << 16), __uint_as_float(u.x & 0xffff0000u), __uint_as_float(u.y << 16),
                       __uint_as_float(u.y & 0xffff0000u));
}
__device__ __forceinline__ void store4(float* p, float4 v) { *reinterpret_cast<float4*>(p) = v; }
__device__ __forceinline__ void store4(bf16_t* p, float4 v) {
    *reinterpret_cast<uint2*>(p) = make_uint2(pack_bf2(v.x, v.y), pack_bf2(v.z, v.w));
}

template <typename TIN, typename TOUT, int NI>
__global__ __launch_bounds__(256) void ln_fwd_kernel(const TIN* __restrict__ x, long long ldx, const float* __restrict__ gamma,
                                                     TOUT* __restrict__ y, long long ldy, bf16_t* __restrict__ xcopy, long long ldc,
                                                     float* __restrict__ mean_out, float* __restrict__ rstd_out, int rows, int D) {
    const int lane = threadIdx.x & 63;
    const int wpb = blockDim.x >> 6;
    for (int row = blockIdx.x * wpb + (threadIdx.x >> 6); row < rows; row += gridDim.x * wpb) {
// ... 9 lines not shown
        float q = 0.f;
#pragma unroll
        for (int i = 0; i < NI; ++i) {
            const int e = (i * 64 + lane) * 4;
            if (e < D) {
                const float a = v[i].x - mean, b = v[i].y - mean, c = v[i].z - mean, d = v[i].w - mean;
                q += a * a + b * b + c * c + d * d;
            }
        }
        const float rstd = rsqrtf(wave_sum(q) / (float)D + LN_EPS);
#pragma unroll
        for (int i = 0; i < NI; ++i) {
            const int e = (i * 64 + lane) * 4;
            if (e < D) {
                const float4 g = load4(gamma + e);
                store4(y + (long long)row * ldy + e,
                       make_float4((v[i].x - mean) * rstd * g.x, (v[i].y - mean) * rstd * g.y, (v[i].z - mean) * rstd * g.z,
                                   (v[i].w - mean) * rstd * g.w));
                if (xcopy) store4(xcopy + (long long)row * ldc + e, v[i]);
            }
        }
        if (lane == 0) {
            mean_out[row] = mean;
            rstd_out[row] = rstd;
        }
    }
}

template <typename TDY, typename TX, typename TDX, int NI>
__global__ __launch_bounds__(256) void ln_bwd_kernel(const TDY* __restrict__ dy, long long lddy, const TX* __restrict__ x, long long ldx,
                                                     const float* __restrict__ mean_in, const float* __restrict__ rstd_in,
                                                     const float* __restrict__ gamma, const bf16_t* __restrict__ extra, long long lde,
                                                     TDX* __restrict__ dx, long long lddx, float* __restrict__ dgamma_part, int rows, int D) {
    __shared__ float red[4][NI * 256];
    const int lane = threadIdx.x & 63, wave = threadIdx.x >> 6;
    float4 dg[NI];
#pragma unroll
    for (int i = 0; i < NI; ++i) dg[i] = make_float4(0.f, 0.f, 0.f, 0.f);
    for (int row = blockIdx.x * 4 + wave; row < rows; row += gridDim.x * 4) {
        const float mean = mean_in[row], rstd = rstd_in[row];
        float4 xh[NI], g[NI];
        float s1 = 0.f, s2 = 0.f;
#pragma unroll
        for (int i = 0; i < NI; ++i) {
            const int e = (i * 64 + lane) * 4;
            if (e < D) {
                const float4 xv = load4(x + (long long)row * ldx + e);
                const float4 d = load4(dy + (long long)row * lddy + e);
                const float4 gm = load4(gamma + e);
                xh[i] = make_float4((xv.x - mean) * rstd, (xv.y - mean) * rstd, (xv.z - mean) * rstd, (xv.w - mean) * rstd);
                g[i] = make_float4(d.x * gm.x, d.y * gm.y, d.z * gm.z, d.w * gm.w);
                dg[i].x += d.x * xh[i].x; dg[i].y += d.y * xh[i].y; dg[i].z += d.z * xh[i].z; dg[i].w += d.w * xh[i].w;
                s1 += g[i].x + g[i].y + g[i].z + g[i].w;
                s2 += g[i].x * xh[i].x + g[i].y * xh[i].y + g[i].z * xh[i].z + g[i].w * xh[i].w;
            } else {
                xh[i] = g[i] = make_float4(0.f, 0.f, 0.f, 0.f);
            }
        }
        const float c1 = wave_sum(s1) / (float)D, c2 = wave_sum(s2) / (float)D;
#pragma unroll
        for (int i = 0; i < NI; ++i) {
            const int e = (i * 64 + lane) * 4;
            if (e < D) {
                float4 o = make_float4(rstd * (g[i].x - c1 - xh[i].x * c2), rstd * (g[i].y - c1 - xh[i].y * c2),
                                       rstd * (g[i].z - c1 - xh[i].z * c2), rstd * (g[i].w - c1 - xh[i].w * c2));
                if (extra) {
                    const float4 ex = load4(extra + (long long)row * lde + e);
                    o.x += ex.x; o.y += ex.y; o.z += ex.z; o.w += ex.w;
                }
                store4(dx + (long long)row * lddx + e, o);
            }
        }
    }
    if (!dgamma_part) return;
#pragma unroll
    for (int i = 0; i < NI; ++i) *reinterpret_cast<float4*>(&red[wave][(i * 64 + lane) * 4]) = dg[i];
    __syncthreads();
    for (int e = threadIdx.x; e < D; e += 256)
        dgamma_part[(long long)blockIdx.x * D + e] = red[0][e] + red[1][e] + red[2][e] + red[3][e];
}

template <typename T>
__global__ __launch_bounds__(256) void colsum_kernel(const T* __restrict__ in, long long ld, int rows, int cols, float* __restrict__ out,
                                                     float scale, int accumulate, int rows_per_chunk, int direct) {
    __shared__ float red[4][64];
    const int cx = threadIdx.x & 63, ry = threadIdx.x >> 6;
    const int c = blockIdx.x * 64 + cx;
    const int r0 = blockIdx.y * rows_per_chunk, r1 = min(rows, r0 + rows_per_chunk);
    float s0 = 0.f, s1 = 0.f, s2 = 0.f, s3 = 0.f;
    auto ldv = [&](int r) -> float {
        if constexpr (sizeof(T) == 2) return bf2f(in[(long long)r * ld + c]);
        else return in[(long long)r * ld + c];
    };
    if (c < cols) {
        int r = r0 + ry;
        for (; r + 12 < r1; r += 16) {
            s0 += ldv(r); s1 += ldv(r + 4); s2 += ldv(r + 8); s3 += ldv(r + 12);
        }
        for (; r < r1; r += 4) s0 += ldv(r);
    }
    red[ry][cx] = (s0 + s1) + (s2 + s3);
    __syncthreads();
    if (ry == 0 && c < cols) {
        const float v = (red[0][cx] + red[1][cx]) + (red[2][cx] + red[3][cx]);
        if (direct) out[c] = accumulate ? out[c] + v * scale : v * scale;
        else out[(long long)blockIdx.y * cols + c] = v;
    }
}

__global__ __launch_bounds__(256) void colsum_finish_kernel(const float* __restrict__ ws, int chunks, int cols, float* __restrict__ out, float scale,
                                                            int accumulate) {
    const int c = blockIdx.x * 256 + threadIdx.x;
    if (c >= cols) return;
    float v = 0.f;
    for (int k = 0; k < chunks; ++k) v += ws[(long long)k * cols + c];
    v *= scale;
    out[c] = accumulate ? out[c] + v : v;
}

__device__ __forceinline__ float& f4e(float4& v, int c) { return reinterpret_cast<float*>(&v)[c]; }
__device__ __forceinline__ float f4e(const float4& v, int c) { return reinterpret_cast<const float*>(&v)[c]; }

constexpr int GE_MAX = 3;

__device__ __forceinline__ float block_sum256(float v, float* red) {
    v = wave_sum(v);
    if ((threadIdx.x & 63) == 0) red[threadIdx.x >> 6] = v;
    __syncthreads();
    return red[0] + red[1] + red[2] + red[3];
}
__device__ __forceinline__ void block_sum256x2(float& a, float& b, float* red) {
    a = wave_sum(a);
    b = wave_sum(b);
    if ((threadIdx.x & 63) == 0) { red[threadIdx.x >> 6] = a; red[4 + (threadIdx.x >> 6)] = b; }
    __syncthreads();
    a = red[0] + red[1] + red[2] + red[3];
    b = red[4] + red[5] + red[6] + red[7];
}

__global__ __launch_bounds__(256) void geglu_ln_fwd_kernel(const bf16_t* __restrict__ u, long long ldu, int goff, const float* __restrict__ gamma,
                                                           bf16_t* __restrict__ out, long long ldo, float* __restrict__ mean_out,
                                                           float* __restrict__ rstd_out, int rows, int I, int Ipad) {
    __shared__ float red[4][4];
    const int t = threadIdx.x;
    float4 gam[GE_MAX];
#pragma unroll
    for (int j = 0; j < GE_MAX; ++j) {
        const int e = (t + 256 * j) * 4;
        gam[j] = make_float4(e < I ? gamma[e] : 0.f, e + 1 < I ? gamma[e + 1] : 0.f, e + 2 < I ? gamma[e + 2] : 0.f, e + 3 < I ? gamma[e + 3] : 0.f);
    }
    struct Raw { uint2 x[GE_MAX], g[GE_MAX]; };
    auto issue = [&](Raw& r, int row) {
#pragma unroll
        for (int j = 0; j < GE_MAX; ++j) {
            const int e = (t + 256 * j) * 4;
            r.x[j] = r.g[j] = make_uint2(0u, 0u);
            if (e < Ipad && row < rows) {
                r.x[j] = *reinterpret_cast<const uint2*>(u + (long long)row * ldu + e);
                r.g[j] = *reinterpret_cast<const uint2*>(u + (long long)row * ldu + goff + e);
            }
        }
    };
    auto cvt = [](uint2 v) {
        return make_float4(__uint_as_float(v.x << 16), __uint_as_float(v.x & 0xffff0000u), __uint_as_float(v.y << 16), __uint_as_float(v.y & 0xffff0000u));
    };
    auto process = [&](const Raw& r, int row, int par) {
        float4 h[GE_MAX];
        float s = 0.f;
#pragma unroll
        for (int j = 0; j < GE_MAX; ++j) {
            const int e = (t + 256 * j) * 4;
            h[j] = make_float4(0.f, 0.f, 0.f, 0.f);
            if (e < Ipad) {
                const float4 xv = cvt(r.x[j]);
                const float4 gv = cvt(r.g[j]);
#pragma unroll
                for (int c = 0; c < 4; ++c) {
                    float cdf, pdf;
                    gauss_cdf_pdf(f4e(gv, c), cdf, pdf);
                    f4e(h[j], c) = (e + c < I) ? f4e(gv, c) * cdf * f4e(xv, c) : 0.f;
                }
                s += h[j].x + h[j].y + h[j].z + h[j].w;
            }
        }
        const float mean = block_sum256(s, red[par]) / (float)I;
        float q = 0.f;
#pragma unroll
        for (int j = 0; j < GE_MAX; ++j) {
            const int e = (t + 256 * j) * 4;
            if (e < I) {
                const float a = h[j].x - mean, b = h[j].y - mean, c = h[j].z - mean, d = h[j].w - mean;
                q += a * a + (e + 1 < I ? b * b : 0.f) + (e + 2 < I ? c * c : 0.f) + (e + 3 < I ? d * d : 0.f);
            }
        }
        const float rstd = rsqrtf(block_sum256(q, red[par + 1]) / (float)I + LN_EPS);
#pragma unroll
// ... 168 lines not shown
        const long long r = e / I;
        const int c = (int)(e % I);
        const float xv = x[r * 2 * I + c], g = x[r * 2 * I + I + c], d = dy[e];
        dx[r * 2 * I + c] = d * gelu_f(g);
        dx[r * 2 * I + I + c] = d * xv * gelu_grad_f(g);
    }
}

}

extern "C" int alm_ln_partial_blocks(int rows) { return min((rows + 3) / 4, 512); }

extern "C" int alm_layernorm_fwd(const void* x, int x_is_bf16, long long ldx, const float* gamma, void* y, int y_is_f32, long long ldy, void* xcopy,
                                 long long ldc, float* mean, float* rstd, int rows, int D, void* stream) {
    if (rows <= 0) return 0;
    if ((D & 3) || (ldx & 3) || (ldy & 3) || (xcopy && (ldc & 3))) return ALM_ERR_BAD_ARG;
    hipStream_t st = (hipStream_t)stream;
    int rc;
    if (y_is_f32)
        rc = x_is_bf16 ? launch_ln_fwd((const bf16_t*)x, ldx, gamma, (float*)y, ldy, (bf16_t*)xcopy, ldc, mean, rstd, rows, D, st)
                       : launch_ln_fwd((const float*)x, ldx, gamma, (float*)y, ldy, (bf16_t*)xcopy, ldc, mean, rstd, rows, D, st);
    else
        rc = x_is_bf16 ? launch_ln_fwd((const bf16_t*)x, ldx, gamma, (bf16_t*)y, ldy, (bf16_t*)xcopy, ldc, mean, rstd, rows, D, st)
                       : launch_ln_fwd((const float*)x, ldx, gamma, (bf16_t*)y, ldy, (bf16_t*)xcopy, ldc, mean, rstd, rows, D, st);
    if (rc) return rc;
    ALM_LAUNCH_CHECK();
    return 0;
}

extern "C" int alm_layernorm_bwd(const void* dy, int dy_is_f32, long long lddy, const void* x, int x_is_bf16, long long ldx, const float* mean,
                                 const float* rstd, const float* gamma, const void* extra, long long lde, void* dx, int dx_is_bf16,
                                 long long lddx, float* dgamma_part, int rows, int D, void* stream) {
    if (rows <= 0) return 0;
    if ((D & 3) || (ldx & 3) || (lddy & 3) || (lddx & 3) || (extra && (lde & 3))) return ALM_ERR_BAD_ARG;
    const int grid = alm_ln_partial_blocks(rows);
    hipStream_t st = (hipStream_t)stream;
    int rc;
    if (dy_is_f32) {
        if (x_is_bf16 || dx_is_bf16) return ALM_ERR_UNSUPPORTED;
        rc = launch_ln_bwd((const float*)dy, lddy, (const float*)x, ldx, mean, rstd, gamma, (const bf16_t*)extra, lde, (float*)dx, lddx, dgamma_part, grid, rows, D, st);
    } else if (x_is_bf16 && dx_is_bf16)
        rc = launch_ln_bwd((const bf16_t*)dy, lddy, (const bf16_t*)x, ldx, mean, rstd, gamma, (const bf16_t*)extra, lde, (bf16_t*)dx, lddx, dgamma_part, grid, rows, D, st);
    else if (x_is_bf16)
        rc = launch_ln_bwd((const bf16_t*)dy, lddy, (const bf16_t*)x, ldx, mean, rstd, gamma, (const bf16_t*)extra, lde, (float*)dx, lddx, dgamma_part, grid, rows, D, st);
    else if (dx_is_bf16)
        rc = launch_ln_bwd((const bf16_t*)dy, lddy, (const float*)x, ldx, mean, rstd, gamma, (const bf16_t*)extra, lde, (bf16_t*)dx, lddx, dgamma_part, grid, rows, D, st);
    else
        rc = launch_ln_bwd((const bf16_t*)dy, lddy, (const float*)x, ldx, mean, rstd, gamma, (const bf16_t*)extra, lde, (float*)dx, lddx, dgamma_part, grid, rows, D, st);
    if (rc) return rc;
    ALM_LAUNCH_CHECK();
    return 0;
}

extern "C" int alm_colsum_chunks(int rows);
extern "C" int alm_colsum_partial(const float* in, long long ld, int rows, int cols, float* ws, void* stream) {
    if (cols <= 0 || rows <= 0 || !ws) return ALM_ERR_BAD_ARG;
    const int chunks = alm_colsum_chunks(rows);
    const int rpc = (rows + chunks - 1) / chunks;
    hipLaunchKernelGGL(colsum_kernel<float>, dim3((cols + 63) / 64, chunks), dim3(256), 0, (hipStream_t)stream, in, ld, rows, cols, ws, 1.f, 0, rpc, 0);
    ALM_LAUNCH_CHECK();
    return 0;
}

extern "C" int alm_colsum_chunks(int rows) { return rows <= 128 ? 1 : min(16, (rows + 63) / 64); }

extern "C" int alm_colsum(const void* in, int in_is_bf16, long long ld, int rows, int cols, float* out, float scale, int accumulate, float* ws,
                          void* stream) {
    if (cols <= 0) return 0;
    const int chunks = ws ? alm_colsum_chunks(rows) : 1;
    const int rpc = (rows + chunks - 1) / chunks;
    const int direct = chunks == 1;
    dim3 grid((cols + 63) / 64, chunks);
    float* o1 = direct ? out : ws;
    if (in_is_bf16)
        hipLaunchKernelGGL(colsum_kernel<bf16_t>, grid, dim3(256), 0, (hipStream_t)stream, (const bf16_t*)in, ld, rows, cols, o1, scale, accumulate, rpc, direct);
    else
        hipLaunchKernelGGL(colsum_kernel<float>, grid, dim3(256), 0, (hipStream_t)stream, (const float*)in, ld, rows, cols, o1, scale, accumulate, rpc, direct);
    if (!direct)
        hipLaunchKernelGGL(colsum_finish_kernel, dim3((cols + 255) / 256), dim3(256), 0, (hipStream_t)stream, ws, chunks, cols, out, scale, accumulate);
    ALM_LAUNCH_CHECK();
    return 0;
}

extern "C" int alm_geglu_partial_blocks(int rows) { return min(rows, 1024); }

extern "C" int alm_geglu_ln_fwd(const void* u, long long ldu, int gate_offset, const float* gamma, void* out, long long ldo, float* mean,
                                float* rstd, int rows, int inner, int inner_pad, void* stream) {
    if (rows <= 0) return 0;
    if (inner <= 0 || inner_pad < inner || inner_pad > GE_MAX * 1024 || (inner_pad & 7) || (ldu & 7) || (gate_offset & 7)) return ALM_ERR_UNSUPPORTED;
    hipLaunchKernelGGL(geglu_ln_fwd_kernel, dim3(min(rows, 2048)), dim3(256), 0, (hipStream_t)stream, (const bf16_t*)u, ldu, gate_offset, gamma,
                       (bf16_t*)out, ldo, mean, rstd, rows, inner, inner_pad);
    ALM_LAUNCH_CHECK();
    return 0;
}

extern "C" int alm_geglu_ln_bwd(const void* dhn, long long lddh, const void* u, long long ldu, int gate_offset, const float* gamma,
                                const float* mean, const float* rstd, void* du, float* dgamma_part, int rows, int inner, int inner_pad,
                                void* stream) {
    if (rows <= 0) return 0;
    if (inner <= 0 || inner_pad < inner || inner_pad > GE_MAX * 1024 || (inner_pad & 7) || (ldu & 7) || (gate_offset & 7)) return ALM_ERR_UNSUPPORTED;
    hipLaunchKernelGGL(geglu_ln_bwd_kernel, dim3(alm_geglu_partial_blocks(rows)), dim3(256), 0, (hipStream_t)stream, (const bf16_t*)dhn, lddh,
                       (const bf16_t*)u, ldu, gate_offset, gamma, mean, rstd, (bf16_t*)du, dgamma_part, rows, inner, inner_pad);
    ALM_LAUNCH_CHECK();
    return 0;
}

extern "C" int alm_geglu_fwd(const float* x, float* y, long long rows, int inner, void* stream) {
    if (rows <= 0 || inner <= 0) return 0;
    const long long n = rows * inner;
    hipLaunchKernelGGL(geglu_fwd_kernel, dim3((unsigned)min((n + 255) / 256, (long long)8192)), dim3(256), 0, (hipStream_t)stream, x, y, rows, inner);
    ALM_LAUNCH_CHECK();
    return 0;
}

extern "C" int alm_geglu_bwd(const float* dy, const float* x, float* dx, long long rows, int inner, void* stream) {
    if (rows <= 0 || inner <= 0) return 0;
    const long long n = rows * inner;
    hipLaunchKernelGGL(geglu_bwd_kernel, dim3((unsigned)min((n + 255) / 256, (long long)8192)), dim3(256), 0, (hipStream_t)stream, dy, x, dx, rows, inner);
    ALM_LAUNCH_CHECK();
    return 0;
}
```

audiolm-pytorch_amd/launchlist.py:

```python
from __future__ import annotations

import bisect
import ctypes
import dataclasses
import math
import os
import struct
import sys

import torch

from . import _lib, ops

ENABLED = os.environ.get('ALM_LAUNCH_LIST', '1') != '0'
MAX_ARENA_BYTES = int(float(os.environ.get('ALM_LAUNCH_LIST_MAX_GB', '24')) * (1 << 30))
MAX_PLANS = max(1, int(os.environ.get('ALM_LAUNCH_LIST_MAX_PLANS', '64')))
ALIGN = 256
LITERAL, STREAM, HOST_PTRS, HOST_INTS = 0, 0xFFFF, 0xFFFE, 0xFFFD
_P, _I, _L, _F, _U = _lib._P, _lib._I, _lib._L, _lib._F, _lib._U
_M64 = (1 << 64) - 1

STATS = dict(sized=0, recorded=0, replayed=0, refused=0)


# ... 145 lines not shown
                elif isinstance(a, ctypes.Array):
                    arrays.append((len(self.slots), a))
                    self.slots.append(0), self.reloc.append(LITERAL)
                elif isinstance(a, int):
                    bid, off = self._classify(a, f'{name} argument {i}')
                    self.slots.append(off), self.reloc.append(bid)
                else:
                    self.fail(f'{name} argument {i}: {type(a).__name__} is not a device pointer')
                    self.slots.append(0), self.reloc.append(LITERAL)
            elif t is _F:
                self.slots.append(struct.unpack('<I', struct.pack('<f', float(a)))[0]), self.reloc.append(LITERAL)
            else:
                self.slots.append(int(a) & _M64), self.reloc.append(LITERAL)
        for at, arr in arrays:
            here = len(self.slots)
            if arr._type_ is ctypes.c_void_p:
                for j, v in enumerate(arr):
                    if v is None:
                        self.slots.append(0), self.reloc.append(LITERAL)
                    else:
                        bid, off = self._classify(int(v), f'{name} host array element {j}')
                        self.slots.append(off), self.reloc.append(bid)
                self.slots[at], self.reloc[at] = here, HOST_PTRS
            elif arr._type_ is ctypes.c_int:
                vals = [int(v) & 0xFFFFFFFF for v in arr] + [0]
                for j in range(0, len(vals) - 1, 2):
                    self.slots.append(vals[j] | (vals[j + 1] << 32)), self.reloc.append(LITERAL)
                self.slots[at], self.reloc[at] = here, HOST_INTS
            else:
                self.fail(f'{name}: host array of {arr._type_.__name__}')
        self.entries.append((op, len(sig), first))
        self.names.append(name)

    def finish(self, arena_bytes):
        rec = Recorded(self.entries, self.slots, self.reloc, self.nbases, arena_bytes)
        rec.names = self.names
        return rec


def _spec(t, arena, rec):
    if t is None:
        return None
    off = t.data_ptr() - arena.base
    if not (0 <= off and off + _extent(t) <= arena.cap) or off % t.element_size():
        rec.fail('an output of the pass does not live in its arena')
        return None
    return (off // t.element_size(), t.dtype, tuple(t.shape), tuple(t.stride()))


def _rebuild(spec, typed):
    if spec is None:
        return None
    off, dtype, shape, stride = spec
    return typed[dtype].as_strided(shape, stride, off)


def _typed(buf):
    return {torch.float32: buf.view(torch.float32), torch.bfloat16: buf.view(torch.bfloat16)}



class Plan:
    def __init__(self, key):
        self.key = key
        self.state = 'size'
        self.fwd_bytes = self.bwd_bytes = None
        self.fwd = self.bwd = None
        self.why = None
        self.dhn_dtype = None
        self.orphans = 0


class Replay:

    def __init__(self, plan, arena, xin):
        self.plan, self.arena, self.xin = plan, arena, xin


PLANS = {}


def _switches(core):
    return (core.QKV_GROUP, core.QKV_GROUP_MAX_M, core.ASYNC_KV, core.DEFER_WGRAD, core.DEFER_GROUPS, core.DEFER_GROUP_SIZES, core.DEFER_MAX_BYTES, core.HC_BATCH_FINISH,
            core.PACK_ALL, core.ASYNC_WGRAD, core.SIDE_STREAMS, ops.NT_WS)


def plan_for(core, x, mask_u8, cfg, need, bias, nflat, defer, dx_scale):
    if not ENABLED:
        return None
    dev = x.device
    key = (dev.index, ops._st(), tuple(x.shape), need, mask_u8 is None, None if bias is None else int(bias.tbl.shape[1]), dataclasses.astuple(cfg), nflat,
           bool(defer), float(dx_scale), _switches(core))
    plan = PLANS.pop(key, None)
    if plan is None:
        plan = Plan(key)
        while len(PLANS) >= MAX_PLANS:
            PLANS.pop(next(iter(PLANS)))
    PLANS[key] = plan
    return None if plan.state == 'off' else plan


def _weight_images(core, cache, cfg):
    out = []
    for l in range(cfg.depth):
        for kind in core.branch_kinds(cfg):
            for name in ('wq', 'wkv', 'wo', 'w1', 'w2'):
                hit = cache.store.get((l, kind, name))
                if hit is not None:
                    out += [hit[1][0], hit[1][1]]
    return out


def _bias_tensors(bias):
    return [] if bias is None else [bias.tbl, bias.qkey4, bias.kkey4, bias.qattr, bias.kattr]


def _turn_off(plan, why):
    plan.state, plan.why, plan.fwd, plan.bwd = 'off', why, None, None
    STATS['refused'] += 1
    print(f'[audiolm_pytorch_amd] launch list refused for a stack shape (the eager path stays in use): {why}', file=sys.stderr, flush=True)


def _fill(rec, first, tensors):
    b = rec.bases
    for i, t in enumerate(tensors, first):
        b[i] = 0 if t is None else t.data_ptr()


def forward(core, plan, xin, mask_u8, flat, cfg, cache, need, bias, defer):
    kw = dict(defer_wgrad=defer)
    if plan.state == 'ready' and (plan.bwd is not None or not need):
        core.pack_stack_weights(cache, flat, cfg)
        rec = plan.fwd
        arena = torch.empty(rec.arena_bytes, dtype=torch.uint8, device=xin.device)
        rec.bases[0] = arena.data_ptr()
        _fill(rec, 1, [xin, mask_u8] + _bias_tensors(bias) + list(flat) + _weight_images(core, cache, cfg))
        rec.run(ops._st())
        STATS['replayed'] += 1
        hn = _rebuild(rec.outputs, _typed(arena))
        return hn, (Replay(plan, arena, xin) if need else None)
    core.pack_stack_weights(cache, flat, cfg)
    if plan.state == 'size':
        tally = _Tally()
        ops.ALLOC = tally
        try:
            hn, saved = core.stack_forward(xin, mask_u8, flat, cfg, cache, need, bias, **kw)
        finally:
            ops.ALLOC = None
        plan.fwd_bytes = tally.bytes
        STATS['sized'] += 1
        if tally.bytes > MAX_ARENA_BYTES:
            _turn_off(plan, f'forward arena of {tally.bytes / 2 ** 30:.1f} GB exceeds ALM_LAUNCH_LIST_MAX_GB')
        elif not need:
            plan.state = 'record'
        if saved is not None:
            saved['_ll'] = (plan, 'size', None, xin)
        return hn, saved
    plan.orphans += 1
    if plan.orphans > 8:
        _turn_off(plan, 'forwards with gradients enabled whose backward never ran')
        return core.stack_forward(xin, mask_u8, flat, cfg, cache, need, bias, **kw)
    bases = [None, xin, mask_u8] + _bias_tensors(bias) + list(flat) + _weight_images(core, cache, cfg)
    arena = _Arena(plan.fwd_bytes, xin.device)
    bases[0] = (arena.base, arena.cap)
    rec = Recorder(bases, ops._st())
    arena.recorder = rec
    ops.ALLOC, _lib.RECORDER = arena, rec
# ... 73 lines not shown
```

audiolm-pytorch_amd/ops.py:

```python
from __future__ import annotations

import ctypes
import os

import torch

from . import _lib

BF16, F32 = torch.bfloat16, torch.float32


_raw_stream = getattr(torch._C, '_cuda_getCurrentRawStream', None)
_cur_dev = getattr(torch._C, '_cuda_getDevice', None) or torch.cuda.current_device


def _st():
    if _raw_stream is not None:
        return _raw_stream(_cur_dev())
    return torch.cuda.current_stream().cuda_stream


def _chk(t, dtype=None):
    if not t.is_cuda:
        raise _lib.AlmError('audiolm_pytorch_amd ops run on the MI355X only (got a CPU tensor); there is no CPU fallback')
    if dtype is not None and t.dtype != dtype:
        raise _lib.AlmError(f'expected {dtype}, got {t.dtype}')
    if t.device.index != _cur_dev():
        raise _lib.AlmError(f'tensor on cuda:{t.device.index} but the current device is cuda:{torch.cuda.current_device()}: call '
                            'torch.cuda.set_device(...) (one process per GPU) before using audiolm_pytorch_amd')
    return t


def _p(t):
    return None if t is None else t.data_ptr()


ALLOC = None


def _new(shape, dtype=None, device=None):
    if ALLOC is not None:
        return ALLOC.empty(shape, dtype, device)
    return torch.empty(shape, dtype=dtype, device=device)


def _new_zeros(shape, dtype=None, device=None):
    if ALLOC is not None:
        return ALLOC.zeros(shape, dtype, device)
    return torch.zeros(shape, dtype=dtype, device=device)


def _new_like(t):
    if ALLOC is not None and t.is_contiguous():
        return ALLOC.empty(t.shape, t.dtype, t.device)
    return torch.empty_like(t)


def memset_zero(t):
    assert t.is_contiguous()
    _lib.call('alm_memset_zero', t.data_ptr(), t.numel() * t.element_size(), _st())
    return t


def persistent_buffers():
    return list(_NT_WS.values())


def _rows_ld(t):
    assert t.dim() == 2 and t.stride(1) == 1, (t.shape, t.stride())
    return t.shape[0], t.shape[1], t.stride(0)



_NT_WS = {}
NT_WS = os.environ.get('ALM_GEMM_NT_WS', '1') != '0'


def _nt_ws(dev, stream):
    key = (dev.index, stream)
    ws = _NT_WS.get(key)
    if ws is None:
        ws = _NT_WS[key] = torch.zeros(_lib.query('alm_gemm_nt_ws_bytes'), dtype=torch.uint8, device=dev)
    return ws


def gemm_nt(A, B, C, *, bias=None, alpha=1.0, accumulate=False):
    _chk(A, BF16), _chk(B, BF16), _chk(C)
    assert A.stride(-1) == 1 and B.stride(-1) == 1 and C.stride(-1) == 1
    nb = A.dim() - 2
    assert nb in (0, 1, 2) and B.dim() == A.dim() and C.dim() == A.dim()
    M, K = A.shape[-2:]
    N = B.shape[-2]
    assert B.shape[-1] == K and C.shape[-2] == M and C.shape[-1] == N, (A.shape, B.shape, C.shape)
    bs = [1, 1]
    sa, sb, sc = [0, 0], [0, 0], [0, 0]
    for i in range(nb):
        j = 2 - nb + i
        bs[j] = A.shape[i]
        sa[j], sb[j], sc[j] = A.stride(i), B.stride(i) if B.shape[i] != 1 else 0, C.stride(i)
    st = _st()
    if NT_WS and M >= 256 and N >= 256:
        ws = _nt_ws(A.device, st)
        _lib.call('alm_gemm_bf16_nt_ws', A.data_ptr(), B.data_ptr(), C.data_ptr(), _p(bias), M, N, K, A.stride(-2), B.stride(-2), C.stride(-2),
                  bs[0], bs[1], sa[0], sa[1], sb[0], sb[1], sc[0], sc[1], float(alpha), int(C.dtype == F32), int(accumulate), ws.data_ptr(), ws.numel(), st)
    else:
        _lib.call('alm_gemm_bf16_nt', A.data_ptr(), B.data_ptr(), C.data_ptr(), _p(bias), M, N, K, A.stride(-2), B.stride(-2), C.stride(-2),
                  bs[0], bs[1], sa[0], sa[1], sb[0], sb[1], sc[0], sc[1], float(alpha), int(C.dtype == F32), int(accumulate), st)
    return C


def gemm_nt_inl(A, B, C, slices, *, bias=None, alpha=1.0, accumulate=False):
    _chk(A, BF16), _chk(B, BF16), _chk(C)
    M, K = A.shape
    N = B.shape[0]
    st = _st()
    ws = _nt_ws(A.device, st)
    _lib.call('alm_gemm_bf16_nt_inl', A.data_ptr(), B.data_ptr(), C.data_ptr(), _p(bias), M, N, K, A.stride(0), B.stride(0), C.stride(0),
              float(alpha), int(C.dtype == F32), int(accumulate), int(slices), ws.data_ptr(), ws.numel(), st)
    return C


def gemm_nt_group2(A0, B0, C0, A1, B1, C1):
    for t in (A0, B0, A1, B1):
        _chk(t, BF16)
        assert t.dim() == 2 and t.stride(1) == 1
    _chk(C0), _chk(C1)
    assert C0.dtype == C1.dtype and C0.stride(1) == 1 and C1.stride(1) == 1
    (M0, K0), (M1, K1), N0, N1 = A0.shape, A1.shape, B0.shape[0], B1.shape[0]
    assert B0.shape[1] == K0 and B1.shape[1] == K1 and tuple(C0.shape) == (M0, N0) and tuple(C1.shape) == (M1, N1)
    _lib.call('alm_gemm_bf16_nt_group2', A0.data_ptr(), B0.data_ptr(), C0.data_ptr(), M0, N0, K0, A0.stride(0), B0.stride(0), C0.stride(0),
              A1.data_ptr(), B1.data_ptr(), C1.data_ptr(), M1, N1, K1, A1.stride(0), B1.stride(0), C1.stride(0), int(C0.dtype == F32), _st())
    return C0, C1


def _splitk(name, A, B, C, M, N, K, nb, sA, sB, sC, alpha, accumulate):
    nws = _lib.query('alm_gemm_splitk_ws_floats', M, N, K, nb)
    if nws < 0:
        raise _lib.AlmError('split-K workspace exceeds 2^31 floats')
    ws = _new(nws, dtype=F32, device=A.device) if nws > 0 else None
    _lib.call(name, A.data_ptr(), B.data_ptr(), C.data_ptr(), _p(ws), M, N, K, A.stride(-2), B.stride(-2), C.stride(-2), nb, sA, sB, sC,
              float(alpha), int(accumulate), _st())
    return C


def gemm_nt_splitk(A, B, C, *, alpha=1.0, accumulate=False):
    _chk(A, BF16), _chk(B, BF16), _chk(C, F32)
    M, K = A.shape
    N = B.shape[0]
# ... 56 lines not shown


def pack_weights_multi(jobs):
    arr = (_lib.AlmPackJob * len(jobs))()
    for i, (w, dst, dstT, rp, cp) in enumerate(jobs):
        _chk(w, F32)
        rows, cols, ld = _rows_ld(w)
        arr[i] = _lib.AlmPackJob(w.data_ptr(), rows, cols, ld, _p(dst), dst.stride(0) if dst is not None else 0, rp, cp,
                                 _p(dstT), dstT.stride(0) if dstT is not None else 0)
    _lib.call('alm_pack_weights_multi', ctypes.cast(arr, ctypes.c_void_p), len(jobs), _st())



def layernorm_fwd(x, gamma, *, want_copy=False, out_f32=False, y_out=None, xc_out=None):
    _chk(x)
    rows, D, ld = _rows_ld(x)
    y = _new((rows, D), dtype=F32 if out_f32 else BF16, device=x.device) if y_out is None else y_out
    xc = (_new((rows, D), dtype=BF16, device=x.device) if xc_out is None else xc_out) if want_copy else None
    assert y.shape == (rows, D) and y.is_contiguous() and (xc is None or (xc.shape == (rows, D) and xc.is_contiguous()))
    mean = _new(rows, dtype=F32, device=x.device)
    rstd = _new(rows, dtype=F32, device=x.device)
    _lib.call('alm_layernorm_fwd', x.data_ptr(), int(x.dtype == BF16), ld, gamma.data_ptr(), y.data_ptr(), int(out_f32), D, _p(xc), D, mean.data_ptr(),
              rstd.data_ptr(), rows, D, _st())
    return y, xc, mean, rstd


def colsum(inp, out=None, scale=1.0, accumulate=False):
    _chk(inp)
    rows, cols, ld = _rows_ld(inp)
    if out is None:
        out = _new(cols, dtype=F32, device=inp.device)
    chunks = _lib.query('alm_colsum_chunks', rows)
    ws = _new((chunks, cols), dtype=F32, device=inp.device) if chunks > 1 else None
    _lib.call('alm_colsum', inp.data_ptr(), int(inp.dtype == BF16), ld, rows, cols, out.data_ptr(), float(scale), int(accumulate), _p(ws), _st())
    return out


def layernorm_bwd(dy, x, mean, rstd, gamma, *, extra=None, dx_dtype=F32, want_dgamma=True):
    _chk(dy), _chk(x)
    assert dy.dtype in (BF16, F32)
    rows, D, lddy = _rows_ld(dy)
    dx = _new((rows, D), dtype=dx_dtype, device=dy.device)
    part = None
    if want_dgamma:
        nblk = _lib.query('alm_ln_partial_blocks', rows)
        part = _new((nblk, D), dtype=F32, device=dy.device)
    _lib.call('alm_layernorm_bwd', dy.data_ptr(), int(dy.dtype == F32), lddy, x.data_ptr(), int(x.dtype == BF16), x.stride(0), mean.data_ptr(), rstd.data_ptr(),
              gamma.data_ptr(), _p(extra), extra.stride(0) if extra is not None else 0, dx.data_ptr(), int(dx_dtype == BF16), D, _p(part),
              rows, D, _st())
    return dx, (colsum(part) if want_dgamma else None)


def geglu_fwd(x):
    _chk(x, F32)
    rows, two_i, ld = _rows_ld(x)
    assert ld == two_i and two_i % 2 == 0
    y = _new((rows, two_i // 2), dtype=F32, device=x.device)
    _lib.call('alm_geglu_fwd', x.data_ptr(), y.data_ptr(), rows, two_i // 2, _st())
    return y


def geglu_bwd(dy, x):
    _chk(dy, F32), _chk(x, F32)
    rows, two_i, ld = _rows_ld(x)
    assert ld == two_i and dy.shape == (rows, two_i // 2) and dy.is_contiguous()
    dx = _new_like(x)
    _lib.call('alm_geglu_bwd', dy.data_ptr(), x.data_ptr(), dx.data_ptr(), rows, two_i // 2, _st())
    return dx


def geglu_ln_fwd(u, gamma, inner, inner_pad, out=None):
    _chk(u, BF16)
    rows, _, ldu = _rows_ld(u)
    if out is None:
        out = _new((rows, inner_pad), dtype=BF16, device=u.device)
    assert out.shape == (rows, inner_pad) and out.dtype == BF16 and out.stride(1) == 1 and out.stride(0) == inner_pad
    mean = _new(rows, dtype=F32, device=u.device)
    rstd = _new(rows, dtype=F32, device=u.device)
    _lib.call('alm_geglu_ln_fwd', u.data_ptr(), ldu, inner_pad, gamma.data_ptr(), out.data_ptr(), inner_pad, mean.data_ptr(), rstd.data_ptr(),
              rows, inner, inner_pad, _st())
    return out, mean, rstd


def geglu_ln_bwd(dhn, u, gamma, mean, rstd, inner, inner_pad, du_out=None):
    rows, _, ldu = _rows_ld(u)
    du = _new_like(u) if du_out is None else du_out
    assert du.shape == u.shape and du.stride(0) == ldu and du.stride(1) == 1 and du.dtype == BF16
    nblk = _lib.query('alm_geglu_partial_blocks', rows)
    part = _new((nblk, inner), dtype=F32, device=u.device)
    _lib.call('alm_geglu_ln_bwd', dhn.data_ptr(), dhn.stride(0), u.data_ptr(), ldu, inner_pad, gamma.data_ptr(), mean.data_ptr(), rstd.data_ptr(),
              du.data_ptr(), part.data_ptr(), rows, inner, inner_pad, _st())
    return du, colsum(part)



def _bias_args(bias, N, H):
    tbl = _chk(bias.tbl, F32)
    assert tbl.dim() == 2 and tbl.shape[0] == H and tbl.is_contiguous(), tbl.shape
    for t in (bias.qkey4, bias.kkey4, bias.qattr, bias.kattr):
        _chk(t, torch.int32)
        assert t.shape == (N,) and t.is_contiguous(), (t.shape, N)
    return (tbl.data_ptr(), tbl.shape[1], bias.qkey4.data_ptr(), bias.kkey4.data_ptr(), bias.qattr.data_ptr(), bias.kattr.data_ptr())


def attn_bias_part(B, N, H, LT, device):
    return _new_zeros((_lib.query('alm_attn_bias_part_rows', B, N, H), LT), dtype=F32, device=device)


def attn_bias_grad_reduce(part, B, N, H, dim_head=64):
    LT = part.shape[1]
    dtbl = _new((H, LT), dtype=F32, device=part.device)
    _lib.call('alm_attn_bias_grad_reduce', part.data_ptr(), dtbl.data_ptr(), B, N, H, LT, float(dim_head) ** -0.5, _st())
    return dtbl


def mqa_attn_fwd(q, k, v, mask, B, N, H, dim_head=64, bias=None, dropout_p=0., seed=0, o=None, seed_dev=None):
    _chk(q, BF16), _chk(k, BF16), _chk(v, BF16)
    if o is None:
        o = _new((B * N, H * dim_head), dtype=BF16, device=q.device)
    assert o.shape == (B * N, H * dim_head) and o.dtype == BF16 and o.stride(1) == 1
    lse = _new((B, H, N), dtype=F32, device=q.device)
    if bias is not None:
        _lib.call('alm_mqa_attn_bias_fwd', q.data_ptr(), q.stride(0), k.data_ptr(), k.stride(0), v.data_ptr(), v.stride(0), _p(mask), o.data_ptr(),
                  o.stride(0), lse.data_ptr(), B, N, H, dim_head, float(dim_head) ** -0.5, *_bias_args(bias, N, H), float(dropout_p), int(seed), _p(seed_dev), _st())
        return o, lse
    _lib.call('alm_mqa_attn_fwd', q.data_ptr(), q.stride(0), k.data_ptr(), k.stride(0), v.data_ptr(), v.stride(0), _p(mask), o.data_ptr(),
              o.stride(0), lse.data_ptr(), B, N, H, dim_head, float(dim_head) ** -0.5, float(dropout_p), int(seed), _p(seed_dev), _st())
    return o, lse


def mqa_attn_bwd(q, k, v, mask, o, lse, dout, B, N, H, dim_head=64, bias=None, dtbl_part=None, dropout_p=0., seed=0, dq_out=None, seed_dev=None):
    _chk(dout, BF16)
    dq = _new_like(q) if dq_out is None else dq_out
    assert dq.shape == q.shape and dq.dtype == BF16 and dq.stride(1) == 1
    hg = _lib.query('alm_mqa_bwd_parts', B, N, H)
    dkv = _new((hg, B * N, 2 * dim_head), dtype=F32, device=q.device)
    delta = _new((2, B, H, N), dtype=F32, device=q.device)
    if bias is not None:
        assert dtbl_part is not None and dtbl_part.shape[1] == bias.tbl.shape[1] and dtbl_part.is_contiguous()
        _lib.call('alm_mqa_attn_bias_bwd', q.data_ptr(), q.stride(0), k.data_ptr(), k.stride(0), v.data_ptr(), v.stride(0), _p(mask),
                  o.data_ptr(), o.stride(0), lse.data_ptr(), dout.data_ptr(), dout.stride(0), dq.data_ptr(), dq.stride(0), dkv.data_ptr(),
                  dkv.data_ptr() + 4 * dim_head, dkv.stride(1), dkv.stride(0), delta.data_ptr(), B, N, H, dim_head, float(dim_head) ** -0.5,
                  *_bias_args(bias, N, H), dtbl_part.data_ptr(), float(dropout_p), int(seed), _p(seed_dev), _st())
        return dq, dkv
    _lib.call('alm_mqa_attn_bwd', q.data_ptr(), q.stride(0), k.data_ptr(), k.stride(0), v.data_ptr(), v.stride(0), _p(mask), o.data_ptr(),
              o.stride(0), lse.data_ptr(), dout.data_ptr(), dout.stride(0), dq.data_ptr(), dq.stride(0), dkv.data_ptr(),
              dkv.data_ptr() + 4 * dim_head, dkv.stride(1), dkv.stride(0), delta.data_ptr(), B, N, H, dim_head, float(dim_head) ** -0.5,
              float(dropout_p), int(seed), _p(seed_dev), _st())
    return dq, dkv


def mqa_decode_attn(q, cache, kv_new, pos, mask, H, dim_head=64, bias=None, pos_dev=None):
    _chk(q, BF16), _chk(cache, BF16), _chk(kv_new, BF16)
    B, Nmax = cache.shape[0], cache.shape[1]
    assert cache.is_contiguous() and cache.shape[2] == 2 * dim_head and kv_new.shape == (B, 2 * dim_head) and kv_new.stride(1) == 1
    out = _new((B, H * dim_head), dtype=BF16, device=q.device)
    qk = qa = 0
    tb = (None, 0)
    vecs = (None, None, None, None)
    if bias is not None:
        tbl = _chk(bias.tbl, F32)
        assert tbl.is_contiguous() and tbl.shape[0] == H and bias.kkey4.shape[0] >= Nmax
        tb = (tbl.data_ptr(), tbl.shape[1])
        if pos_dev is None:
            qk, qa = int(bias.qkey4_host[pos]), int(bias.qattr_host[pos])
        vecs = (bias.kkey4.data_ptr(), bias.kattr.data_ptr(), bias.qkey4.data_ptr(), bias.qattr.data_ptr())
    _lib.call('alm_mqa_decode_attn', q.data_ptr(), q.stride(0), cache.data_ptr(), cache.stride(0), kv_new.data_ptr(), kv_new.stride(0), _p(mask),
              mask.stride(0) if mask is not None else 0, out.data_ptr(), out.stride(0), B, H, dim_head, int(pos), Nmax, float(dim_head) ** -0.5,
              tb[0], tb[1], qk, qa, vecs[0], vecs[1], _p(pos_dev), vecs[2] if pos_dev is not None else None,
              vecs[3] if pos_dev is not None else None, _st())
    return out


def value_residual_mix(v, v0):
    rows, dh, _ = _rows_ld(v)
    out = _new((rows, dh), dtype=BF16, device=v.device)
    _lib.call('alm_value_residual_mix', v.data_ptr(), v.stride(0), v0.data_ptr(), v0.stride(0), out.data_ptr(), dh, rows, dh, _st())
    return out


def loss_combine(sums, labels, weights, ignore_index=-1):
    G = len(sums)
    assert 1 <= G <= 4 and len(labels) == G and len(weights) == G
    dev = sums[0].device
    labels = [l if l.is_contiguous() else l.contiguous() for l in labels]
    for t, l in zip(sums, labels):
        _chk(t, F32)
        _chk(l, torch.int64)
    loss = _new(1, dtype=F32, device=dev)
    scales = _new(G, dtype=F32, device=dev)
    pad = [None] * (4 - G)
    _lib.call('alm_loss_combine', *[t.data_ptr() for t in sums], *pad, *[l.data_ptr() for l in labels], *pad, *[l.numel() for l in labels], *([0] * (4 - G)),
              *[float(w) for w in weights], *([0.0] * (4 - G)), G, int(ignore_index), loss.data_ptr(), scales.data_ptr(), _st())
    return loss, scales


def coarse_prepare(sem, coarse, pad_id, sem_eos, coarse_eos, Q, C, sem_has_eos=False):
    _chk(sem, torch.int64), _chk(coarse, torch.int64)
    assert sem.dim() == 2 and coarse.dim() == 2 and sem.stride(1) == 1 and coarse.stride(1) == 1 and sem.shape[0] == coarse.shape[0]
    B, ns0 = sem.shape
    nc0 = coarse.shape[1]
    ns = ns0 + (0 if sem_has_eos else 1)
    N, dev = ns + nc0 + 2, sem.device
    sl = _new((B, ns), dtype=torch.int64, device=dev)
    cl = _new((B, nc0 + 1), dtype=torch.int64, device=dev)
    src_a = _new((B, N), dtype=torch.int32, device=dev)
    keep = _new((B, N), dtype=torch.bool, device=dev)
    _lib.call('alm_coarse_prepare', sem.data_ptr(), sem.stride(0), coarse.data_ptr(), coarse.stride(0), B, ns0, nc0, int(pad_id), int(sem_eos), int(coarse_eos),
              int(Q), int(C), sl.data_ptr(), cl.data_ptr(), src_a.data_ptr(), keep.data_ptr(), 1 if sem_has_eos else 0, _st())
    return sl, cl, src_a, keep


def semantic_prepare(sem, eos_id, num_rows, has_eos=False):
    _chk(sem, torch.int64)
    assert sem.dim() == 2 and (sem.shape[1] == 0 or sem.stride(1) == 1)
    B, n0 = sem.shape
    W = n0 + (0 if has_eos else 1)
    labels = _new((B, W), dtype=torch.int64, device=sem.device)
    src_a = _new((B, W), dtype=torch.int32, device=sem.device)
    _lib.call('alm_semantic_prepare', sem.data_ptr(), sem.stride(0), B, n0, int(eos_id), int(num_rows), labels.data_ptr(), src_a.data_ptr(), 1 if has_eos else 0, _st())
    return labels, src_a


def unique_consecutive(ids, eos_id=None, pad=-1):
    _chk(ids, torch.int64)
    assert ids.dim() == 2 and (ids.shape[1] == 0 or ids.stride(1) == 1)
# ... 713 lines not shown
```

include/audiolm_hip.h:

```cpp
#pragma once
#ifdef __cplusplus
extern "C" {
#endif

#define ALM_ERR_BAD_ARG 10001
#define ALM_ERR_UNSUPPORTED 10002

int alm_gemm_bf16_nt(const void* A, const void* B, void* C, const float* bias, int M, int N, int K, long long lda, long long ldb,
                     long long ldc, int nb1, int nb2, long long sA1, long long sA2, long long sB1, long long sB2, long long sC1,
                     long long sC2, float alpha, int out_f32, int accumulate, void* stream);
int alm_gemm_bf16_nt_ws(const void* A, const void* B, void* C, const float* bias, int M, int N, int K, long long lda, long long ldb, long long ldc,
                        int nb1, int nb2, long long sA1, long long sA2, long long sB1, long long sB2, long long sC1, long long sC2, float alpha,
                        int out_f32, int accumulate, void* ws, long long ws_bytes, void* stream);
int alm_gemm_bf16_nt_inl(const void* A, const void* B, void* C, const float* bias, int M, int N, int K, long long lda, long long ldb, long long ldc,
                         float alpha, int out_f32, int accumulate, int slices, void* ws, long long ws_bytes, void* stream);
int alm_gemm_nt_plan(int M, int N, int K, int nb, int with_ws, int* plan);
int alm_gemm_nt_ws_bytes(void);
int alm_gemm_bf16_nt_group2(const void* A0, const void* B0, void* C0, int M0, int N0, int K0, long long lda0, long long ldb0, long long ldc0,
                            const void* A1, const void* B1, void* C1, int M1, int N1, int K1, long long lda1, long long ldb1, long long ldc1,
                            int out_f32, void* stream);
int alm_gemm_bf16_nt_tile(const void* A, const void* B, void* C, const float* bias, int M, int N, int K, long long lda, long long ldb,
                          long long ldc, float alpha, int out_f32, int accumulate, int tile, void* stream);
int alm_gemm_splitk_slices(int M, int N, int K, int nb);
int alm_gemm_splitk_ws_floats(int M, int N, int K, int nb);
int alm_gemm_splitk_tile(int M, int N, int K, int nb);
int alm_gemm_nt_tile_choice(int M, int N, int nb);
int alm_gemm_tn_batched_plan(int M, int N, int K, int nb, int* plan);
int alm_gemm_bf16_nt_splitk(const void* A, const void* B, float* C, float* ws, int M, int N, int K, long long lda, long long ldb,
                            long long ldc, int nb, long long sA, long long sB, long long sC, float alpha, int accumulate, void* stream);
int alm_gemm_bf16_tn_splitk(const void* At, const void* Bt, float* C, float* ws, int M, int N, int K, long long lda, long long ldb,
                            long long ldc, int nb, long long sA, long long sB, long long sC, float alpha, int accumulate, void* stream);
int alm_gemm_bf16_tn_batched(const void* At, const void* Bt, float* C, float* ws, int M, int N, int K, long long lda, long long ldb, long long ldc,
                             int nb1, int nb2, long long sA1, long long sA2, long long sB1, long long sB2, long long sC1, long long sC2, float alpha,
                             int accumulate, void* stream);
int alm_transpose_bf16(const void* src, void* dst, int rows, int cols, long long ld_src, long long ld_dst, int rows_pad, void* stream);
int alm_transpose_bf16_batched(const void* src, void* dst, int rows, int cols, long long ld_src, long long ld_dst, int rows_pad, int nb,
                               long long bs_src, long long bs_dst, void* stream);
int alm_pack_weight(const float* src, int rows, int cols, long long ld_src, void* dst, long long ld_dst, int rows_pad, int cols_pad,
                    void* dstT, long long ld_dstT, void* stream);

typedef struct {
    const float* src; int rows, cols; long long ld_src;
    void* dst; long long ld_dst; int rows_pad, cols_pad;
    void* dstT; long long ld_dstT;
} AlmPackJob;
int alm_pack_weights_multi(const AlmPackJob* jobs, int njobs, void* stream);

int alm_ln_partial_blocks(int rows);
int alm_layernorm_fwd(const void* x, int x_is_bf16, long long ldx, const float* gamma, void* y, int y_is_f32, long long ldy, void* xcopy_bf16,
                      long long ldc, float* mean, float* rstd, int rows, int D, void* stream);
int alm_layernorm_bwd(const void* dy, int dy_is_f32, long long lddy, const void* x, int x_is_bf16, long long ldx, const float* mean,
                      const float* rstd, const float* gamma, const void* extra_bf16, long long lde, void* dx, int dx_is_bf16,
                      long long lddx, float* dgamma_part, int rows, int D, void* stream);
int alm_colsum(const void* in, int in_is_bf16, long long ld, int rows, int cols, float* out, float scale, int accumulate, float* ws,
               void* stream);
int alm_colsum_chunks(int rows);
int alm_colsum_partial(const float* in, long long ld, int rows, int cols, float* ws, void* stream);

int alm_geglu_fwd(const float* x, float* y, long long rows, int inner, void* stream);
int alm_geglu_bwd(const float* dy, const float* x, float* dx, long long rows, int inner, void* stream);
int alm_geglu_partial_blocks(int rows);
int alm_geglu_ln_fwd(const void* u_bf16, long long ldu, int gate_offset, const float* gamma, void* out_bf16, long long ldo, float* mean,
                     float* rstd, int rows, int inner, int inner_pad, void* stream);
int alm_geglu_ln_bwd(const void* dhn_bf16, long long lddh, const void* u_bf16, long long ldu, int gate_offset, const float* gamma,
                     const float* mean, const float* rstd, void* du_bf16, float* dgamma_part, int rows, int inner, int inner_pad,
                     void* stream);

int alm_mqa_attn_fwd(const void* q, long long ldq, const void* k, long long ldk, const void* v, long long ldv, const unsigned char* mask,
                     void* o, long long ldo, float* lse, int B, int N, int H, int dim_head, float scale, float dropout_p,
                     unsigned long long seed, const void* seed_dev, void* stream);
int alm_mqa_attn_bwd(const void* q, long long ldq, const void* k, long long ldk, const void* v, long long ldv, const unsigned char* mask,
                     const void* o, long long ldo, const float* lse, const void* dout, long long lddo, void* dq, long long lddq, float* dk,
                     float* dv, long long lddk, long long part_stride, float* delta, int B, int N, int H, int dim_head, float scale,
                     float dropout_p, unsigned long long seed, const void* seed_dev, void* stream);
int alm_mqa_head_groups(int H);
int alm_mqa_bwd_parts(int B, int N, int H);
int alm_mqa_attn_bias_fwd(const void* q, long long ldq, const void* k, long long ldk, const void* v, long long ldv, const unsigned char* mask,
                          void* o, long long ldo, float* lse, int B, int N, int H, int dim_head, float scale, const float* tbl, int LT,
                          const int* qkey4, const int* kkey4, const int* qattr, const int* kattr, float dropout_p, unsigned long long seed,
                          const void* seed_dev, void* stream);
int alm_mqa_attn_bias_bwd(const void* q, long long ldq, const void* k, long long ldk, const void* v, long long ldv, const unsigned char* mask,
                          const void* o, long long ldo, const float* lse, const void* dout, long long lddo, void* dq, long long lddq,
                          float* dk, float* dv, long long lddk, long long part_stride, float* delta, int B, int N, int H, int dim_head,
                          float scale, const float* tbl, int LT, const int* qkey4, const int* kkey4, const int* qattr, const int* kattr,
                          float* dtbl_part, float dropout_p, unsigned long long seed, const void* seed_dev, void* stream);
int alm_attn_bias_part_rows(int B, int N, int H);
int alm_attn_bias_grad_reduce(const float* dtbl_part, float* dtbl, int B, int N, int H, int LT, float scale, void* stream);
int alm_posmlp_in_fwd(const float* x, const float* W, const float* b, float* pre, void* act_bf16, int L, int in_dim, int C, void* stream);
int alm_posmlp_in_bwd_chunks(int L);
int alm_posmlp_in_bwd(const void* dpre_bf16, const float* x, float* partial, int L, int in_dim, int C, void* stream);
int alm_silu_fwd(const float* pre, void* act_bf16, long long n, void* stream);
int alm_silu_bwd(const float* dact, const float* pre, void* dpre_bf16, long long n, void* stream);
int alm_posmlp_out_fwd(const void* act_bf16, const float* W, const float* b, const float* special, float* tbl, int L, int C, int H,
                       float inv_scale, void* stream);
int alm_posmlp_out_bwd(const float* dtbl, const float* W, const float* pre, void* g_bf16, void* dpre_bf16, float* dspecial, int L, int C, int H,
                       int Hp, float inv_scale, void* stream);
int alm_xattn_softmax_fwd(const float* S, long long ldS, const unsigned char* emask, const float* lse_self, float scale, void* P_bf16, long long ldP,
                          float* lse_tot, float* fself, const float* bias, long long ldbias, int causal_off, int B, int N, int H, int Me, void* stream);
int alm_xattn_dbias(const void* P_bf16, long long ldP, const float* dP, long long lddP, const float* ndelta, float* dbias, long long lddb, int Me, int B,
                    int N, int H, void* stream);
int alm_xattn_combine(const void* o_self_bf16, long long ldos, const float* fself, const float* o_e, void* out_bf16, long long ldo, long long tokens,
                      int H, int dim_head, void* stream);
int alm_xattn_softmax_bwd(const void* P_bf16, long long ldP, const float* dP, long long lddP, const float* ndelta, float scale, void* dS_bf16,
                          long long lddS, int Me, int B, int N, int H, void* stream);
int alm_xattn_delta(const void* o_bf16, long long ldo, const void* dout_bf16, long long lddo, float* ndelta, int B, int N, int H, int dim_head,
                    void* stream);
int alm_value_residual_mix(const void* v, long long ldv, const void* v0, long long ldv0, void* out, long long ldo, long long rows,
                           int dim_head, void* stream);
int alm_kv_grad_pack(const float* dk, const float* dv, long long ld, int nparts, long long part_stride, float* acc_v0, void* dkv_bf16,
                     long long ldo, long long rows, int dim_head, int mode, void* stream);

int alm_loss_combine(const float* s0, const float* s1, const float* s2, const float* s3, const long long* l0, const long long* l1, const long long* l2,
                     const long long* l3, long long n0, long long n1, long long n2, long long n3, float w0, float w1, float w2, float w3, int G,
                     long long ignore_index, float* loss, float* scales, void* stream);

int alm_coarse_prepare(const long long* sem, long long ld_sem, const long long* coarse, long long ld_coarse, int B, int ns0, int nc0, long long pad_id,
                       long long sem_eos, long long coarse_eos, int Q, int C, long long* sem_labels, long long* coarse_labels, int* src_a, void* keep,
                       int sem_has_eos, void* stream);
int alm_semantic_prepare(const long long* sem, long long ld_sem, int B, int n0, long long eos_id, long long num_rows, long long* labels, int* src_a,
                         int has_eos, void* stream);
int alm_unique_consecutive_i64(const long long* ids, long long ld, int B, int n, int append_eos, long long eos_id, long long pad, long long* out,
                               long long ld_out, int* lengths, void* stream);
int alm_fine_prepare(const long long* coarse, long long ld_coarse, const long long* fine, long long ld_fine, int B, int n, int nf, long long pad_id,
                     long long eos_id, int Qc, int Qf, int C, int* src_a, void* keep, void* stream);

int alm_forgetful_mask(const float* score, long long ld_score, void* keep, long long ld_keep, int B, int N, int drop, void* stream);

int alm_hc_coef_width(int S);
int alm_hc_partial_width(int S, int D);
int alm_hc_grads_width(int S, int D);
int alm_hc_partial_rows(int mode, int fused_ln, int r_bf16, int S, long long tokens, int D);
int alm_hc_fwd(const void* R_in, int rin_bcast, int r_bf16, const void* y_prev_bf16, long long ldy, const float* coef_prev, void* R_out,
               const float* hc_gamma, const float* Wa, const float* sa, const float* Aa, const float* wb, const float* sb, const float* Bb,
               const float* ln_gamma, void* x_out_bf16, long long ldx, void* xn_out_bf16, long long ldxn, float* xn32_out, float* mean,
               float* rstd, float* coef, float* xs_out, int mode, int B, int S, int N, int D, void* stream);
int alm_hc_bwd(const void* dRn, int dRn_bcast, int r_bf16, const float* dx, long long lddx, const void* dxn_bf16, long long lddxn,
               const void* extra_bf16, long long ldex, const float* mean, const float* rstd, const float* ln_gamma, const void* R, int r_bcast,
               const float* coef, const float* dbeta, const float* hc_gamma, const float* Wa, const float* sa, const float* wb, const float* sb,
               void* dR, float* dsum, float dsum_scale, float* partial, const void* y_prev_bf16, long long ldy, const float* coef_prev, void* dy_bf16, long long lddy,
               float* dbeta_out, int mode, int B, int S, int N, int D, void* stream);
int alm_hc_param_grads(const float* sums, int chunks, const float* hc_gamma, const float* Wa, const float* wb, float* out, int S, int D, void* stream);
int alm_hc_param_grads_batched(const float* const* parts, const int* rows, int nb, const float* const* gammas, const float* const* Was,
                               const float* const* wbs, float* ws, float* const* outs, int S, int D, void* stream);
int alm_streams_expand(const float* x, float* R, int B, int S, long long nd, void* stream);
int alm_streams_reduce(const float* R, float* x, int B, int S, long long nd, void* stream);
int alm_residual_add(const float* x, const void* y_bf16, long long ldy, float* out, long long rows, int D, void* stream);
int alm_f32_to_bf16(const float* a, const float* b_or_null, void* out_bf16, long long ldo, long long rows, int D, void* stream);
int alm_add_f32(const float* a, const float* b, float* out, long long n, float scale, void* stream);

int alm_embed_assemble(const float* const* tables, const int* table_rows, int ntables, const int* src_a, const int* src_b, float* out,
                       long long rows, int D, int* err_flag, void* stream);
int alm_embed_scatter_add(float* const* grad_tables, const int* table_rows, int ntables, const int* src_a, const int* src_b, const float* dout,
                          float alpha, long long rows, int D, void* stream);
int alm_embed_scatter_ws_floats(const int* table_rows, int ntables, long long rows, int D);
int alm_embed_scatter_owned(float* const* grad_tables, const int* table_rows, int ntables, const int* src_a, const int* src_b, const float* dout,
                            float alpha, long long rows, int D, float* ws, void* stream);
int alm_gather_rows_bf16(const void* in, long long ld_in, const int* idx, void* out, long long ld_out, long long rows, int D, void* stream);
// ... 92 lines not shown
```

Baseline: 1.418 million audio-tokens/s.

## Fuse attention-backward delta and KV-grad pack; batch GEGLU-LN gamma colsums

```diff
diff --git a/audiolm-pytorch_amd/_lib.py b/audiolm-pytorch_amd/_lib.py
--- a/audiolm-pytorch_amd/_lib.py
+++ b/audiolm-pytorch_amd/_lib.py
@@ -35,6 +35,7 @@
     'alm_colsum': [_P, _I, _L, _I, _I, _P, _F, _I, _P, _P],
     'alm_colsum_chunks': [_I],
     'alm_colsum_partial': [_P, _L, _I, _I, _P, _P],
+    'alm_colsum_batched': [_P, _L, _L, _I, _I, _I, _P, _L, _P, _P],
     'alm_geglu_fwd': [_P, _P, _L, _I, _P],
     'alm_geglu_bwd': [_P, _P, _P, _L, _I, _P],
     'alm_geglu_partial_blocks': [_I],
@@ -69,6 +70,8 @@
     'alm_loss_combine': [_P, _P, _P, _P, _P, _P, _P, _P, _L, _L, _L, _L, _F, _F, _F, _F, _I, _L, _P, _P, _P],
     'alm_mqa_head_groups': [_I],
     'alm_mqa_bwd_parts': [_I, _I, _I],
+    'alm_mqa_attn_bwd_fused': [_P, _L, _P, _L, _P, _L, _P, _P, _L, _P, _P, _L, _P, _L, _P, _P, _L, _L, _P, _I, _I, _I, _I, _F, _F, _U, _P, _P, _P, _L, _I, _P, _P],
+    'alm_mqa_bwd_fused_pack': [_I, _I, _I],
     'alm_hc_coef_width': [_I],
     'alm_hc_partial_width': [_I, _I],
     'alm_hc_grads_width': [_I, _I],
diff --git a/audiolm-pytorch_amd/core.py b/audiolm-pytorch_amd/core.py
--- a/audiolm-pytorch_amd/core.py
+++ b/audiolm-pytorch_amd/core.py
@@ -568,6 +568,7 @@
     gsz = (L + ngroups - 1) // ngroups
     return list(range(0, L, gsz))
 HC_BATCH_FINISH = os.environ.get('ALM_HC_BATCH_FINISH', '1') != '0'
+G3_BATCH_FINISH = os.environ.get('ALM_G3_BATCH_FINISH', '1') != '0'
 DEFER_SMALL_LATE = os.environ.get('ALM_DEFER_SMALL_LATE', '1') != '0'
 _DEBUG_DEFER_GROUPS_CAPTURE = 1
 MICRO_ASYNC_WGRAD = os.environ.get('ALM_MICRO_ASYNC_WGRAD', '0') != '0'
@@ -581,7 +582,7 @@
     return 0 if acc is None else (1 if mixed else 2)
 
 
-def ff_backward(cfg, W, prm, sv, dY, side, want_trace=False, du_out=None):
+def ff_backward(cfg, W, prm, sv, dY, side, want_trace=False, du_out=None, g3_part_out=None):
     M, D = dY.shape
     I, Ip, dev = cfg.inner, cfg.inner_pad, dY.device
     (_, W1T), (_, W2T) = W['w1'], W['w2']
@@ -597,7 +598,7 @@
         dW2 = _empty((D, I), F32, dev)
         HNs, dYs = sv['HN'], dY
         run(lambda: ops.gemm_tn_splitk(dYs, HNs[:, :I], dW2, alpha=fa), dYs, HNs, dW2)
-    dU, dg3 = ops.geglu_ln_bwd(dHN, sv['U'], prm['ln3'], sv['mean3'], sv['rstd3'], I, Ip, du_out=du_out)
+    dU, dg3 = ops.geglu_ln_bwd(dHN, sv['U'], prm['ln3'], sv['mean3'], sv['rstd3'], I, Ip, du_out=du_out, part_out=g3_part_out)
     dXN = _empty((M, D), BF16, dev)
     ops.gemm_nt(dU, W1T, dXN)
     dW1 = None
@@ -731,6 +732,20 @@
                 rec_['hc_grads'] = dict(g_)
         hc_pending.clear()
 
+    g3_parts = _empty((cfg.depth, ops.geglu_partial_blocks(M), I), F32, dev) if (wg is not None and G3_BATCH_FINISH) else None
+    g3_pending = []
+
+    def finish_g3():
+        if not g3_pending:
+            return
+        lo, hi = min(t[0] for t in g3_pending), max(t[0] for t in g3_pending)
+        sums = ops.colsum_batched(g3_parts[lo:hi + 1])
+        for l_, gi_, rec_ in g3_pending:
+            grads[gi_] = sums[l_ - lo]
+            if rec_ is not None:
+                rec_['dg3'] = grads[gi_]
+        g3_pending.clear()
+
     def add_ctx(g):
         nonlocal dctx
         dctx = g if dctx is None else ops.add_f32(dctx, g)
@@ -751,9 +766,12 @@
         extra = None
         W = LW[kind]
         if kind == 'ff':
-            dXN, dW1, dg3, dW2, dHN, dU = ff_backward(cfg, W, prm, sv, dY, side, want_trace=True, du_out=bst['dU'][l] if bst is not None else None)
+            dXN, dW1, dg3, dW2, dHN, dU = ff_backward(cfg, W, prm, sv, dY, side, want_trace=True, du_out=bst['dU'][l] if bst is not None else None,
+                                                      g3_part_out=g3_parts[l] if g3_parts is not None else None)
             grads[ip + 1], grads[ip + 2], grads[ip + 3] = dW1, dg3, dW2
             rec = dict(dY=dY, dHN=dHN, dU=dU, dXN=dXN, dW1=dW1, dg3=dg3, dW2=dW2) if TRACE is not None else None
+            if g3_parts is not None:
+                g3_pending.append((l, ip + 2, rec))
         elif kind == 'cross':
             (_, WqT), (_, WkvT), (_, WoT) = W['wq'], W['wkv'], W['wo']
             m = ctx.m
@@ -808,9 +826,14 @@
                     dke, dve = dke[:, mpre:], dve[:, mpre:]
                 dkv32 = torch.cat((dke.reshape(M, dh), dve.reshape(M, dh)), dim=1).contiguous()
             else:
+                pack = dict(acc=acc_v0, mode=_vgrad_mode(acc_v0, sv['mixed']), out=bst['dKV'][l] if bst is not None else None) if bias is None else None
                 dQ, dkv32 = ops.mqa_attn_bwd(sv['Q'], KV[:, :dh], sv['V'], mask_u8, sv['AO'], sv['LSE'], dAO, B, N, H, dh, bias=bias, dtbl_part=dtbl_part,
-                                             dropout_p=pd, seed=dseed, dq_out=bst['dQ'][l] if bst is not None else None, seed_dev=dseed_dev)
-            dKV = ops.kv_grad_pack(dkv32, acc_v0, _vgrad_mode(acc_v0, sv['mixed']), dh, out=bst['dKV'][l] if bst is not None else None)
+                                             dropout_p=pd, seed=dseed, dq_out=bst['dQ'][l] if bst is not None else None, seed_dev=dseed_dev,
+                                             fused=bias is None, pack=pack)
+            if not dense and pack is not None and pack['done']:
+                dKV = pack['out']
+            else:
+                dKV = ops.kv_grad_pack(dkv32, acc_v0, _vgrad_mode(acc_v0, sv['mixed']), dh, out=bst['dKV'][l] if bst is not None else None)
             dKVp = None
             pre = sv['pre']
             if pre is not None:
@@ -871,12 +894,14 @@
         sv.clear()
         if wg is not None and (prev is None or prev['layer'] != l) and l in starts:
             finish_hc()
+            finish_g3()
             launch_group(l)
         if on_layer_grads is not None and wg is None and (prev is None or prev['layer'] != l):
             base = l * ppl
             side.run_after_all(lambda: on_layer_grads(l, grads[base:base + ppl]), *[g for g in grads[base:base + ppl] if g is not None])
 
     finish_hc()
+    finish_g3()
     dx = dR.view(B, N, D)
     dtbl = ddense if dense else (ops.attn_bias_grad_reduce(dtbl_part, B, N, H) if bias is not None else None)
     side.join()
diff --git a/audiolm-pytorch_amd/csrc/attention.hip b/audiolm-pytorch_amd/csrc/attention.hip
--- a/audiolm-pytorch_amd/csrc/attention.hip
+++ b/audiolm-pytorch_amd/csrc/attention.hip
@@ -84,6 +84,11 @@
     int LT;
     unsigned drop_thr; float drop_scale; unsigned seed_lo, seed_hi;
     const unsigned long long* seed_dev;
+    float* delta_out; float* nlse_out;
+    float inv_scale;
+    bf16_t* pack_out; long long ld_pack;
+    float* acc_v0; int vmode;
+    unsigned* tickets;
 };
 
 __device__ __forceinline__ unsigned mix32(unsigned x) {
@@ -550,7 +555,26 @@
             dof[qb][ks] = gload8(dp + ks * 16 + lh * 8, ok);
         }
         lse2[qb] = ok ? lse_log2(p.lse[((long long)b * p.H + head) * p.N + qi]) : INFINITY;
-        dlt[qb] = ok ? p.ndelta[((long long)b * p.H + head) * p.N + qi] : 0.f;
+        if (!BIAS && p.delta_out) {
+            const bf16_t* op = p.o + ((long long)b * p.N + qi) * p.ldo + head * DH;
+            float s = 0.f;
+#pragma unroll
+            for (int ks = 0; ks < 4; ++ks) {
+                const bf16x8 of = gload8(op + ks * 16 + lh * 8, ok);
+#pragma unroll
+                for (int j = 0; j < 8; ++j) s += bf2f((bf16_t)of[j]) * bf2f((bf16_t)dof[qb][ks][j]);
+            }
+            s += __shfl_xor(s, 32, 64);
+            dlt[qb] = -s;
+            if (ok && lh == 0) {
+                const long long idx = ((long long)b * p.H + head) * p.N + qi;
+                p.delta_out[idx] = -s;
+                const float l = p.lse[idx];
+                p.nlse_out[idx] = (l == -INFINITY) ? -INFINITY : -l * p.inv_scale;
+            }
+        } else {
+            dlt[qb] = ok ? p.ndelta[((long long)b * p.H + head) * p.N + qi] : 0.f;
+        }
     }
 
     int kq4[2] = {0, 0}, aq[2] = {0, 0}, qmin4[2] = {0, 0}, qmax4[2] = {0, 0};
@@ -1093,9 +1117,44 @@
             for (int hh = 0; hh < nh; ++hh) sum += red[(hh * 2 + half) * RW + d * RS + kl];
             if (kblk * 64 + kk < p.N) {
                 const bool kv_ok = !p.mask || p.mask[(long long)b * p.N + kblk * 64 + kk] != 0;
-                outp[((long long)b * p.N + kblk * 64 + kk) * p.lddk + d] = kv_ok ? sum * sc : 0.f;
-            }
-        }
+                float* dst = outp + ((long long)b * p.N + kblk * 64 + kk) * p.lddk + d;
+                const float val = kv_ok ? sum * sc : 0.f;
+                if (p.pack_out) __hip_atomic_store(dst, val, __ATOMIC_RELAXED, __HIP_MEMORY_SCOPE_AGENT);
+                else *dst = val;
+            }
+        }
+    }
+    if (!p.pack_out) return;
+    asm volatile("s_waitcnt vmcnt(0)" ::: "memory");
+    __syncthreads();
+    unsigned* const flag = reinterpret_cast<unsigned*>(smem);
+    if (t == 0) {
+        unsigned* const cnt = p.tickets + (long long)b * nkb + kblk;
+        const unsigned old = __hip_atomic_fetch_add(cnt, 1u, __ATOMIC_RELAXED, __HIP_MEMORY_SCOPE_AGENT);
+        const unsigned last = old == 1u;
+        if (last) __hip_atomic_store(cnt, 0u, __ATOMIC_RELAXED, __HIP_MEMORY_SCOPE_AGENT);
+        *flag = last;
+    }
+    __syncthreads();
+    if (*flag == 0) return;
+    for (int e = t; e < 64 * 64; e += NT) {
+        const int kk = e >> 6, d = e & 63;
+        if (kblk * 64 + kk >= p.N) continue;
+        const long long r = (long long)b * p.N + kblk * 64 + kk;
+        float gk = 0.f, gv = 0.f;
+#pragma unroll
+        for (int pt = 0; pt < 2; ++pt) {
+            gk += __hip_atomic_load(p.dk + pt * p.part_stride + r * p.lddk + d, __ATOMIC_RELAXED, __HIP_MEMORY_SCOPE_AGENT);
+            gv += __hip_atomic_load(p.dv + pt * p.part_stride + r * p.lddk + d, __ATOMIC_RELAXED, __HIP_MEMORY_SCOPE_AGENT);
+        }
+        if (p.vmode == 1) {
+            gv *= 0.5f;
+            p.acc_v0[r * DH + d] += gv;
+        } else if (p.vmode == 2) {
+            gv += p.acc_v0[r * DH + d];
+        }
+        p.pack_out[r * p.ld_pack + d] = f2bf(gk);
+        p.pack_out[r * p.ld_pack + DH + d] = f2bf(gv);
     }
 }
 
@@ -1200,10 +1259,13 @@
     return 0;
 }
 
+struct FusedArgs { bool on; float* acc_v0; void* dkv; long long ld_dkv; int vmode; unsigned* tickets; };
+
 static int attn_bwd_impl(const void* q, long long ldq, const void* k, long long ldk, const void* v, long long ldv,
                          const unsigned char* mask, const void* o, long long ldo, const float* lse, const void* dout, long long lddo,
                          void* dq, long long lddq, float* dk, float* dv, long long lddk, long long part_stride, float* delta, int B,
-                         int N, int H, int dim_head, float scale, const BiasArgs& ba, float dropout_p, unsigned long long seed, const void* seed_dev, void* stream) {
+                         int N, int H, int dim_head, float scale, const BiasArgs& ba, float dropout_p, unsigned long long seed, const void* seed_dev, void* stream,
+                         const FusedArgs& fa = FusedArgs{false, nullptr, nullptr, 0, 0, nullptr}) {
     if (dim_head != DH) return ALM_ERR_UNSUPPORTED;
     if (dropout_p < 0.f || dropout_p >= 1.f) return ALM_ERR_BAD_ARG;
     int rc = check_attn(B, N, H, ldq, ldk, ldv, ldo);
@@ -1216,9 +1278,13 @@
     hipStream_t st = (hipStream_t)stream;
     float* ndelta = delta;
     float* nlse = delta + (long long)B * H * N;
-    hipLaunchKernelGGL(attn_delta_kernel, dim3(((long long)B * N + 3) / 4), dim3(256), 0, st, (const bf16_t*)o, ldo, (const bf16_t*)dout, lddo, lse,
-                       ndelta, nlse, 1.0f / scale, B, N, H);
+    const bool fuse_delta = fa.on && !ba.tbl;
+    if (fuse_delta && ((uintptr_t)o & 15)) return ALM_ERR_BAD_ARG;
+    if (!fuse_delta)
+        hipLaunchKernelGGL(attn_delta_kernel, dim3(((long long)B * N + 3) / 4), dim3(256), 0, st, (const bf16_t*)o, ldo, (const bf16_t*)dout, lddo, lse,
+                           ndelta, nlse, 1.0f / scale, B, N, H);
     AttnParams p{};
+    if (fuse_delta) { p.o = (bf16_t*)const_cast<void*>(o); p.delta_out = ndelta; p.nlse_out = nlse; p.inv_scale = 1.0f / scale; }
     p.q = (const bf16_t*)q; p.k = (const bf16_t*)k; p.v = (const bf16_t*)v; p.mask = mask; p.lse = const_cast<float*>(lse);
     p.dout = (const bf16_t*)dout; p.ndelta = ndelta; p.nlse = nlse; p.dq = (bf16_t*)dq; p.dk = dk; p.dv = dv;
     p.ldq = ldq; p.ldk = ldk; p.ldv = ldv; p.ldo = ldo; p.lddo = lddo; p.lddq = lddq; p.lddk = lddk; p.part_stride = part_stride;
@@ -1234,6 +1300,11 @@
     const int nh = dkv_heads_per_block(B, N, H);
     p.HG = (H + nh - 1) / nh;
     p.dkv_split = dkv_split(B, N, H, nh);
+    p.delta_out = nullptr; p.nlse_out = nullptr;
+    if (fa.on && fa.dkv) {
+        if (p.HG * p.dkv_split != 2 || !fa.tickets || (long long)B * nqb > 1024 || fa.vmode < 0 || fa.vmode > 2 || (fa.vmode && !fa.acc_v0)) return ALM_ERR_BAD_ARG;
+        p.pack_out = (bf16_t*)fa.dkv; p.ld_pack = fa.ld_dkv; p.acc_v0 = fa.acc_v0; p.vmode = fa.vmode; p.tickets = fa.tickets;
+    }
     auto launch_dkv = [&](auto kern, int threads, int lds) -> hipError_t {
         static const void* done[8] = {nullptr, nullptr, nullptr, nullptr, nullptr, nullptr, nullptr, nullptr};
         const void* fn = reinterpret_cast<const void*>(kern);
@@ -1276,6 +1347,17 @@
                          scale, BiasArgs{}, dropout_p, seed, seed_dev, stream);
 }
 
+extern "C" int alm_mqa_bwd_fused_pack(int B, int N, int H) { return alm_mqa_bwd_parts(B, N, H) == 2 && (long long)B * ((N + 63) / 64) <= 1024 ? 1 : 0; }
+
+extern "C" int alm_mqa_attn_bwd_fused(const void* q, long long ldq, const void* k, long long ldk, const void* v, long long ldv,
+                                      const unsigned char* mask, const void* o, long long ldo, const float* lse, const void* dout, long long lddo,
+                                      void* dq, long long lddq, float* dk, float* dv, long long lddk, long long part_stride, float* delta, int B,
+                                      int N, int H, int dim_head, float scale, float dropout_p, unsigned long long seed, const void* seed_dev,
+                                      float* acc_v0, void* dkv, long long ld_dkv, int vmode, void* tickets, void* stream) {
+    return attn_bwd_impl(q, ldq, k, ldk, v, ldv, mask, o, ldo, lse, dout, lddo, dq, lddq, dk, dv, lddk, part_stride, delta, B, N, H, dim_head,
+                         scale, BiasArgs{}, dropout_p, seed, seed_dev, stream, FusedArgs{true, acc_v0, dkv, ld_dkv, vmode, (unsigned*)tickets});
+}
+
 extern "C" int alm_mqa_attn_bias_fwd(const void* q, long long ldq, const void* k, long long ldk, const void* v, long long ldv,
                                      const unsigned char* mask, void* o, long long ldo, float* lse, int B, int N, int H, int dim_head,
                                      float scale, const float* tbl, int LT, const int* qkey4, const int* kkey4, const int* qattr,
diff --git a/audiolm-pytorch_amd/csrc/launchlist.hip b/audiolm-pytorch_amd/csrc/launchlist.hip
--- a/audiolm-pytorch_amd/csrc/launchlist.hip
+++ b/audiolm-pytorch_amd/csrc/launchlist.hip
@@ -60,10 +60,12 @@
     ALM_OP(alm_layernorm_bwd),
     ALM_OP(alm_colsum),
     ALM_OP(alm_colsum_partial),
+    ALM_OP(alm_colsum_batched),
     ALM_OP(alm_geglu_ln_fwd),
     ALM_OP(alm_geglu_ln_bwd),
     ALM_OP(alm_mqa_attn_fwd),
     ALM_OP(alm_mqa_attn_bwd),
+    ALM_OP(alm_mqa_attn_bwd_fused),
     ALM_OP(alm_mqa_attn_bias_fwd),
     ALM_OP(alm_mqa_attn_bias_bwd),
     ALM_OP(alm_attn_bias_grad_reduce),
diff --git a/audiolm-pytorch_amd/csrc/norm_act.hip b/audiolm-pytorch_amd/csrc/norm_act.hip
--- a/audiolm-pytorch_amd/csrc/norm_act.hip
+++ b/audiolm-pytorch_amd/csrc/norm_act.hip
@@ -115,8 +115,11 @@
 
 template <typename T>
 __global__ __launch_bounds__(256) void colsum_kernel(const T* __restrict__ in, long long ld, int rows, int cols, float* __restrict__ out,
-                                                     float scale, int accumulate, int rows_per_chunk, int direct) {
+                                                     float scale, int accumulate, int rows_per_chunk, int direct, long long in_bs = 0,
+                                                     long long out_bs = 0) {
     __shared__ float red[4][64];
+    in += (long long)blockIdx.z * in_bs;
+    out += (long long)blockIdx.z * out_bs;
     const int cx = threadIdx.x & 63, ry = threadIdx.x >> 6;
     const int c = blockIdx.x * 64 + cx;
     const int r0 = blockIdx.y * rows_per_chunk, r1 = min(rows, r0 + rows_per_chunk);
@@ -142,9 +145,11 @@
 }
 
 __global__ __launch_bounds__(256) void colsum_finish_kernel(const float* __restrict__ ws, int chunks, int cols, float* __restrict__ out, float scale,
-                                                            int accumulate) {
+                                                            int accumulate, long long ws_bs = 0, long long out_bs = 0) {
     const int c = blockIdx.x * 256 + threadIdx.x;
     if (c >= cols) return;
+    ws += (long long)blockIdx.y * ws_bs;
+    out += (long long)blockIdx.y * out_bs;
     float v = 0.f;
     for (int k = 0; k < chunks; ++k) v += ws[(long long)k * cols + c];
     v *= scale;
@@ -479,6 +484,23 @@
     return 0;
 }
 
+extern "C" int alm_colsum_batched(const float* in, long long ld, long long in_bs, int nb, int rows, int cols, float* out, long long out_bs, float* ws,
+                                  void* stream) {
+    if (cols <= 0 || nb <= 0) return 0;
+    if (rows <= 0 || nb > 65535 || !in || !out) return ALM_ERR_BAD_ARG;
+    const int chunks = alm_colsum_chunks(rows);
+    if (chunks > 1 && !ws) return ALM_ERR_BAD_ARG;
+    const int rpc = (rows + chunks - 1) / chunks;
+    const int direct = chunks == 1;
+    hipLaunchKernelGGL(colsum_kernel<float>, dim3((cols + 63) / 64, chunks, nb), dim3(256), 0, (hipStream_t)stream, in, ld, rows, cols, direct ? out : ws, 1.f, 0,
+                       rpc, direct, in_bs, direct ? out_bs : (long long)chunks * cols);
+    if (!direct)
+        hipLaunchKernelGGL(colsum_finish_kernel, dim3((cols + 255) / 256, nb), dim3(256), 0, (hipStream_t)stream, (const float*)ws, chunks, cols, out, 1.f, 0,
+                           (long long)chunks * cols, out_bs);
+    ALM_LAUNCH_CHECK();
+    return 0;
+}
+
 extern "C" int alm_geglu_partial_blocks(int rows) { return min(rows, 1024); }
 
 extern "C" int alm_geglu_ln_fwd(const void* u, long long ldu, int gate_offset, const float* gamma, void* out, long long ldo, float* mean,
diff --git a/audiolm-pytorch_amd/launchlist.py b/audiolm-pytorch_amd/launchlist.py
--- a/audiolm-pytorch_amd/launchlist.py
+++ b/audiolm-pytorch_amd/launchlist.py
@@ -251,7 +251,7 @@
 
 def _switches(core):
     return (core.QKV_GROUP, core.QKV_GROUP_MAX_M, core.ASYNC_KV, core.DEFER_WGRAD, core.DEFER_GROUPS, core.DEFER_GROUP_SIZES, core.DEFER_MAX_BYTES, core.HC_BATCH_FINISH,
-            core.PACK_ALL, core.ASYNC_WGRAD, core.SIDE_STREAMS, ops.NT_WS)
+            core.PACK_ALL, core.ASYNC_WGRAD, core.SIDE_STREAMS, ops.NT_WS, getattr(core, 'G3_BATCH_FINISH', None), ops.ATTN_BWD_FUSED)
 
 
 def plan_for(core, x, mask_u8, cfg, need, bias, nflat, defer, dx_scale):
diff --git a/audiolm-pytorch_amd/ops.py b/audiolm-pytorch_amd/ops.py
--- a/audiolm-pytorch_amd/ops.py
+++ b/audiolm-pytorch_amd/ops.py
@@ -63,7 +63,7 @@
 
 
 def persistent_buffers():
-    return list(_NT_WS.values())
+    return list(_NT_WS.values()) + list(_ATTN_TICKETS.values())
 
 
 def _rows_ld(t):
@@ -286,15 +286,31 @@
     return out, mean, rstd
 
 
-def geglu_ln_bwd(dhn, u, gamma, mean, rstd, inner, inner_pad, du_out=None):
+def geglu_partial_blocks(rows):
+    return _lib.query('alm_geglu_partial_blocks', rows)
+
+
+def geglu_ln_bwd(dhn, u, gamma, mean, rstd, inner, inner_pad, du_out=None, part_out=None):
     rows, _, ldu = _rows_ld(u)
     du = _new_like(u) if du_out is None else du_out
     assert du.shape == u.shape and du.stride(0) == ldu and du.stride(1) == 1 and du.dtype == BF16
     nblk = _lib.query('alm_geglu_partial_blocks', rows)
-    part = _new((nblk, inner), dtype=F32, device=u.device)
+    part = _new((nblk, inner), dtype=F32, device=u.device) if part_out is None else part_out
+    assert part.shape == (nblk, inner) and part.dtype == F32 and part.is_contiguous()
     _lib.call('alm_geglu_ln_bwd', dhn.data_ptr(), dhn.stride(0), u.data_ptr(), ldu, inner_pad, gamma.data_ptr(), mean.data_ptr(), rstd.data_ptr(),
               du.data_ptr(), part.data_ptr(), rows, inner, inner_pad, _st())
-    return du, colsum(part)
+    return du, (colsum(part) if part_out is None else None)
+
+
+def colsum_batched(parts):
+    _chk(parts, F32)
+    assert parts.dim() == 3 and parts.stride(2) == 1
+    nb, rows, cols = parts.shape
+    out = _new((nb, cols), dtype=F32, device=parts.device)
+    chunks = _lib.query('alm_colsum_chunks', rows)
+    ws = _new((nb, chunks, cols), dtype=F32, device=parts.device) if chunks > 1 else None
+    _lib.call('alm_colsum_batched', parts.data_ptr(), parts.stride(1), parts.stride(0), nb, rows, cols, out.data_ptr(), cols, _p(ws), _st())
+    return out
 
 
 
@@ -333,19 +349,53 @@
     return o, lse
 
 
-def mqa_attn_bwd(q, k, v, mask, o, lse, dout, B, N, H, dim_head=64, bias=None, dtbl_part=None, dropout_p=0., seed=0, dq_out=None, seed_dev=None):
+ATTN_BWD_FUSED = os.environ.get('ALM_ATTN_BWD_FUSED', '1') != '0'
+_ATTN_TICKETS = {}
+
+
+def _attn_tickets(dev, stream):
+    key = (dev.index, stream)
+    t = _ATTN_TICKETS.get(key)
+    if t is None:
+        t = _ATTN_TICKETS[key] = torch.zeros(1024, dtype=torch.int32, device=dev)
+    return t
+
+
+def mqa_attn_bwd(q, k, v, mask, o, lse, dout, B, N, H, dim_head=64, bias=None, dtbl_part=None, dropout_p=0., seed=0, dq_out=None, seed_dev=None, *,
+                 fused=False, pack=None, delta_out=None):
     _chk(dout, BF16)
+    if pack is not None:
+        pack['done'] = False
     dq = _new_like(q) if dq_out is None else dq_out
     assert dq.shape == q.shape and dq.dtype == BF16 and dq.stride(1) == 1
     hg = _lib.query('alm_mqa_bwd_parts', B, N, H)
     dkv = _new((hg, B * N, 2 * dim_head), dtype=F32, device=q.device)
-    delta = _new((2, B, H, N), dtype=F32, device=q.device)
+    delta = _new((2, B, H, N), dtype=F32, device=q.device) if delta_out is None else delta_out
+    assert delta.shape == (2, B, H, N) and delta.dtype == F32 and delta.is_contiguous()
     if bias is not None:
         assert dtbl_part is not None and dtbl_part.shape[1] == bias.tbl.shape[1] and dtbl_part.is_contiguous()
         _lib.call('alm_mqa_attn_bias_bwd', q.data_ptr(), q.stride(0), k.data_ptr(), k.stride(0), v.data_ptr(), v.stride(0), _p(mask),
                   o.data_ptr(), o.stride(0), lse.data_ptr(), dout.data_ptr(), dout.stride(0), dq.data_ptr(), dq.stride(0), dkv.data_ptr(),
                   dkv.data_ptr() + 4 * dim_head, dkv.stride(1), dkv.stride(0), delta.data_ptr(), B, N, H, dim_head, float(dim_head) ** -0.5,
                   *_bias_args(bias, N, H), dtbl_part.data_ptr(), float(dropout_p), int(seed), _p(seed_dev), _st())
+        return dq, dkv
+    if fused and ATTN_BWD_FUSED:
+        st = _st()
+        acc = out = tick = None
+        vmode = 0
+        if pack is not None and _lib.query('alm_mqa_bwd_fused_pack', B, N, H):
+            acc, vmode = pack.get('acc'), int(pack['mode'])
+            out = pack.get('out')
+            if out is None:
+                out = pack['out'] = _new((B * N, 2 * dim_head), dtype=BF16, device=q.device)
+            assert out.shape == (B * N, 2 * dim_head) and out.dtype == BF16 and out.stride(1) == 1
+            assert acc is None or (acc.dtype == F32 and acc.shape == (B * N, dim_head) and acc.is_contiguous())
+            tick = _attn_tickets(q.device, st)
+            pack['done'] = True
+        _lib.call('alm_mqa_attn_bwd_fused', q.data_ptr(), q.stride(0), k.data_ptr(), k.stride(0), v.data_ptr(), v.stride(0), _p(mask), o.data_ptr(),
+                  o.stride(0), lse.data_ptr(), dout.data_ptr(), dout.stride(0), dq.data_ptr(), dq.stride(0), dkv.data_ptr(),
+                  dkv.data_ptr() + 4 * dim_head, dkv.stride(1), dkv.stride(0), delta.data_ptr(), B, N, H, dim_head, float(dim_head) ** -0.5,
+                  float(dropout_p), int(seed), _p(seed_dev), _p(acc), _p(out), out.stride(0) if out is not None else 0, vmode, _p(tick), st)
         return dq, dkv
     _lib.call('alm_mqa_attn_bwd', q.data_ptr(), q.stride(0), k.data_ptr(), k.stride(0), v.data_ptr(), v.stride(0), _p(mask), o.data_ptr(),
               o.stride(0), lse.data_ptr(), dout.data_ptr(), dout.stride(0), dq.data_ptr(), dq.stride(0), dkv.data_ptr(),
diff --git a/include/audiolm_hip.h b/include/audiolm_hip.h
--- a/include/audiolm_hip.h
+++ b/include/audiolm_hip.h
@@ -56,6 +56,7 @@
                void* stream);
 int alm_colsum_chunks(int rows);
 int alm_colsum_partial(const float* in, long long ld, int rows, int cols, float* ws, void* stream);
+int alm_colsum_batched(const float* in, long long ld, long long in_bs, int nb, int rows, int cols, float* out, long long out_bs, float* ws, void* stream);
 
 int alm_geglu_fwd(const float* x, float* y, long long rows, int inner, void* stream);
 int alm_geglu_bwd(const float* dy, const float* x, float* dx, long long rows, int inner, void* stream);
@@ -73,6 +74,12 @@
                      const void* o, long long ldo, const float* lse, const void* dout, long long lddo, void* dq, long long lddq, float* dk,
                      float* dv, long long lddk, long long part_stride, float* delta, int B, int N, int H, int dim_head, float scale,
                      float dropout_p, unsigned long long seed, const void* seed_dev, void* stream);
+int alm_mqa_attn_bwd_fused(const void* q, long long ldq, const void* k, long long ldk, const void* v, long long ldv, const unsigned char* mask,
+                           const void* o, long long ldo, const float* lse, const void* dout, long long lddo, void* dq, long long lddq, float* dk,
+                           float* dv, long long lddk, long long part_stride, float* delta, int B, int N, int H, int dim_head, float scale,
+                           float dropout_p, unsigned long long seed, const void* seed_dev, float* acc_v0, void* dkv, long long ld_dkv, int vmode,
+                           void* tickets, void* stream);
+int alm_mqa_bwd_fused_pack(int B, int N, int H);
 int alm_mqa_head_groups(int H);
 int alm_mqa_bwd_parts(int B, int N, int H);
 int alm_mqa_attn_bias_fwd(const void* q, long long ldq, const void* k, long long ldk, const void* v, long long ldv, const unsigned char* mask,
```

Measured after the change: 1.419 million audio-tokens/s (median of 3 runs). No clear change (+0.1%).
